# url-kaist/Quatro

Hardware: AMD Instinct MI355X
Metric: scan-pair registrations/sec (KITTI 64-ch, ~5k corr) + rot/trans err vs ref (higher is better)
Workload: dtype f32 (voxel grid, FPFH, 33-D matching: f16-split MFMA filter, exact f32 decision) / f64 (consistency graph, GNC-TLS, COTE); 1 GPU; composite: qtr_register_pair_corr per step on a synthetic KITTI-64-shaped scan pair (voxel 0.3 m), back end on 5000 planted correspondences, one pair at a time, inputs resident in HBM (--full: the detailed description)

## Files before the change

### include/quatro_hip.h

```cpp
#ifndef QUATRO_HIP_H
#define QUATRO_HIP_H

#include <stddef.h>
#include <stdint.h>

#ifdef __cplusplus
extern "C" {
#endif

#if defined(__GNUC__)
#define QTR_API __attribute__((visibility("default")))
#else
#define QTR_API
#endif

#define QTR_OK 0
#define QTR_ERR_BAD_ARG 1
#define QTR_ERR_CLIQUE_TOO_SMALL 2
#define QTR_ERR_CAPACITY 3
#define QTR_ERR_HIP 4
#define QTR_ERR_UNSUPPORTED 5
#define QTR_ERR_IO 6
#define QTR_ERR_NOT_RUN 7

// ... 286 lines not shown
QTR_API int qtr_place_index_get_info(const qtr_place_index* index, qtr_place_index_info* info);
QTR_API int qtr_place_describe(qtr_handle* h, int slot, const qtr_place_params* params, const float* xyz4, int n, float* desc,
                               int mem);
QTR_API int qtr_place_index_add(qtr_handle* h, int slot, qtr_place_index* index, const qtr_keyframe* kf, int* id_out);
QTR_API int qtr_place_index_add_desc(qtr_handle* h, int slot, qtr_place_index* index, const float* desc, int mem, int* id_out);
QTR_API long long qtr_place_index_fetch(qtr_handle* h, const qtr_place_index* index, int id, int what, void* dst, size_t bytes);
QTR_API int qtr_place_query(qtr_handle* h, int slot, const qtr_place_index* index, const qtr_keyframe* query, int id_lo,
                            int id_hi, int k, qtr_place_match* out, int* n_out);
QTR_API int qtr_place_query_desc(qtr_handle* h, int slot, const qtr_place_index* index, const float* desc, int mem, int id_lo,
                                 int id_hi, int k, qtr_place_match* out, int* n_out);

#define QTR_EVAL_MAX_PAIRS 64
typedef struct qtr_eval_params {
  double max_correspondence_distance;
  int reserved[2];
} qtr_eval_params;
typedef struct qtr_eval_result {
  int status, valid, n_source, n_corr, n_plane, reserved;
  double T[16];
  double overlap, sum_d2, inlier_rmse, plane_rmse, information[36], hessian_plane[36];
} qtr_eval_result;
typedef struct qtr_eval_kf_pair {
  const qtr_keyframe* source;
  const qtr_keyframe* target;
  double T[16];
} qtr_eval_kf_pair;
QTR_API void qtr_default_eval_params(qtr_eval_params* p);
QTR_API int qtr_evaluate(qtr_handle* h, int slot, const float* src4, int n_s, const float* tgt4, int n_t,
                         const float* tgt_normals4, const double T[16], const qtr_eval_params* prm, qtr_eval_result* res, int mem);
QTR_API int qtr_evaluate_pair(qtr_handle* h, int slot, const double T[16], const qtr_eval_params* prm, qtr_eval_result* res);
QTR_API int qtr_evaluate_keyframes(qtr_handle* h, int slot, const qtr_keyframe* source, const qtr_keyframe* target,
                                   const double T[16], const qtr_eval_params* prm, qtr_eval_result* res);
QTR_API int qtr_evaluate_keyframes_batch(qtr_handle* h, int slot, const qtr_eval_kf_pair* pairs, int B,
                                         const qtr_eval_params* prm, qtr_eval_result* results);

#define QTR_PGO_MAX_NODES 65536
#define QTR_PGO_MAX_EDGES (1 << 20)
#define QTR_PGO_MAX_ITERATIONS 65536
#define QTR_PGO_STOP_MAX_ITERATIONS 1
#define QTR_PGO_STOP_RELATIVE 2
#define QTR_PGO_STOP_STEP 3
#define QTR_PGO_STOP_LAMBDA 4
#define QTR_PGO_STOP_NOTHING 5
typedef struct qtr_pgo_params {
  int max_iterations;
  int pcg_max_iterations;
  double rel_tol;
  double step_tol;
  double tau;
  double pcg_tol;
  double line_process_weight;
  double edge_prune_threshold;
  int reserved[8];
} qtr_pgo_params;
typedef struct qtr_pgo_result {
  int status, valid, iterations, accepted, pcg_iterations_total, stop_reason, n_pruned, reserved;
  double objective_initial, objective_final, lambda_final;
} qtr_pgo_result;
QTR_API void qtr_default_pgo_params(qtr_pgo_params* p);
QTR_API int qtr_pgo_optimize(qtr_handle* h, int slot, int n_nodes, const double* poses, const unsigned char* fixed, int n_edges,
                             const int* src, const int* dst, const double* Z, const double* info,
                             const unsigned char* uncertain, const qtr_pgo_params* prm, double* poses_out, double* weight_out,
                             qtr_pgo_result* res);

#define QTR_DBG_GRAPH_BITMAP 1
#define QTR_DBG_CORE 2
#define QTR_DBG_PERM 3
#define QTR_DBG_NBR_OFFSETS 4
#define QTR_DBG_NBR_INDEX 5
#define QTR_DBG_NBR_DIST2 6
#define QTR_DBG_SPFH 7
#define QTR_DBG_NN_LARGE_OF_SMALL 8
#define QTR_DBG_NN_SMALL_OF_LARGE 9
#define QTR_DBG_VOX_SRC 10
#define QTR_DBG_VOX_TGT 11
#define QTR_DBG_CORR 12
#define QTR_DBG_MATCH_STATS 13
#define QTR_DBG_SOLVER_STATE 14
#define QTR_DBG_ICP_CORR 15
#define QTR_DBG_ICP_TRACE 16
#define QTR_DBG_ICP_TIMES 17
#define QTR_DBG_EVAL_CORR 18
#define QTR_DBG_PGO_TRACE 19
QTR_API long long qtr_debug_fetch(qtr_handle* h, int slot, int what, void* dst, size_t bytes);

QTR_API int qtr_debug_math(qtr_handle* h, int fn, const float* a, const float* b, float* out, int n);

#ifdef __cplusplus
}
#endif
#endif
```

### quatro_amd/csrc/capi.hip

```cpp
#include <dlfcn.h>

#include <algorithm>
#include <atomic>
#include <memory>
#include <mutex>
#include <new>
#include <thread>
#include <vector>

#include "common.h"
#include "frontend.h"
#include "solver.h"

struct RcclIdByValue {
  char internal[QTR_COMM_ID_BYTES];
};

struct Slot {
  hipStream_t stream = nullptr;
  hipStream_t stream2 = nullptr;
  hipEvent_t ev[8] = {};
  hipEvent_t ev_vox = nullptr;
  hipStream_t stream3 = nullptr;
  hipEvent_t ev_be0 = nullptr;
  hipEvent_t ev_end = nullptr;
  hipEvent_t ev_fork = nullptr;
  hipEvent_t ev_join = nullptr;
  void* solver_arena = nullptr;
  void* front_arena = nullptr;
  SolverBufs sb;
  FrontBufs fb;
  float4* in_src = nullptr;
  float4* in_tgt = nullptr;
  float4* m_src = nullptr;
  float4* m_tgt = nullptr;
  int* pinned_i32 = nullptr;
  qtr_result* pinned_res = nullptr;
  SegBufs seg;
  void* seg_arena = nullptr;
  ExactBufs exb;
  void* ex_arena = nullptr;
  size_t ex_bytes = 0;
  PwBufs pwb;
  void* pw_arena = nullptr;
  int* mail = nullptr;
  int seq = 0;
  unsigned long long exact_nodes = 0;
  int exact_aborted = 0;
  int times_pending = 0;
  int nn_pending = 0;
  int nn_timed_last = 0;
  long long n_matches = 0;
  float nn_dir_ms[2] = {0, 0};
  double nn_total_ms = 0;
  long long nn_total_launches = 0;
  qtr_stage_times times = {};
  int last_L = 0;
  int last_Wb = 0;
  int last_n = 0;
  int last_ns = 0, last_nt = 0;
  IcpBufs icp;
  EvalBufs eval;
  PgoBufs pgo;
  int reg_ready = 0;
  double reg_T[16] = {};
  int icp_ns = 0, icp_iters = 0;
  float icp_ms[2] = {0, 0};
  PlaceScratch place;
  KfGatherMember* merge_pin = nullptr;
  KfGatherMember* merge_dev = nullptr;
};

enum LanePhase { LANE_IDLE = 0, LANE_VOXELS, LANE_MATCH, LANE_SOLVE, LANE_REFINE_BOXES, LANE_REFINE_ITER };

struct Lane {
  int first_slot = 0, cap = 0;
  ViewStage stage;
  LanePhase phase = LANE_IDLE;
  int first_pair = 0, count = 0;
  std::vector<int> active;
  std::vector<int> ns, nt, L;
  std::vector<int> corr_only;
  std::vector<const float4*> csrc, ctgt;
  std::vector<const float4*> raw_s, raw_t;
  std::vector<int> Ps, Pt;
  bool long_lists = false;
  std::vector<IcpView> iv;
  const IcpView* ref_views = nullptr;
  int ref_it = 0, ref_nchunk = 1;
};
struct qtr_keyframe {
  qtr_handle* owner = nullptr;
  void* dev = nullptr;
  qtr_keyframe_info info = {};
};

struct qtr_place_index {
  qtr_handle* owner = nullptr;
  float* dev = nullptr;
  int stride = 0;
  qtr_place_index_info info = {};
};

struct qtr_voxel_map;

struct BatchJob {
  const qtr_pair_desc* pairs = nullptr;
  int B = 0, next = 0, done = 0;
  qtr_frontend_params fp;
  qtr_params prm;
  qtr_result* results = nullptr;
  int mem = QTR_MEM_HOST;
  bool active = false;
  std::vector<unsigned char> finished;
  bool refine = false;
  qtr_icp_params icp;
  qtr_icp_result* refined = nullptr;
  std::vector<unsigned char> ref_state;
  bool kf = false;
  std::vector<qtr_pair_desc> kf_shadow;
};

struct qtr_handle {
  int device = 0;
  qtr_limits lim;
  std::vector<Slot> slots;
  std::vector<Lane> lanes;
  BatchJob job;
  void* comm = nullptr;
  int comm_rank = 0, comm_world = 1;
  void* comm_buf = nullptr;
  size_t comm_bytes = 0;
  std::atomic<int> solves_in_flight{0};
  int spin_wait = 1;
  bool pre_on = false;
  qtr_pw_params pre_pw;
  qtr_ip_params pre_ip;
  std::atomic<bool> long_lists{false};
  struct Callers {
    std::atomic<int> live{0};
  };
  std::shared_ptr<Callers> callers = std::make_shared<Callers>();
  std::mutex share_mu;
  int share_val = 1, share_gen = 0;
  std::atomic<int> gen_inflight[4] = {};
  unsigned long long uid = 0;
  int stage_events = 1;
  int corr_overlap = 1;
  int nn_event_stride = 1;
  int icp_block = 0;
  std::mutex kf_mu;
  std::vector<qtr_keyframe*> keyframes;
  std::vector<qtr_place_index*> place_indexes;
// ... 375 lines not shown
}

int qtr_create(int device, const qtr_limits* limits, qtr_handle** out) {
  if (!out) return QTR_ERR_BAD_ARG;
  *out = nullptr;
  qtr_handle* h = new (std::nothrow) qtr_handle();
  if (!h) return QTR_ERR_CAPACITY;
  h->err[0] = 0;
  h->device = device;
  h->uid = g_handle_uid.fetch_add(1, std::memory_order_relaxed) + 1;
  {
    const char* hw = getenv("QTR_HOST_WAIT");
    h->spin_wait = (hw && strcmp(hw, "block") == 0) ? 0 : 1;
    const char* se = getenv("QTR_STAGE_EVENTS");
    h->stage_events = (se && atoi(se) == 0) ? 0 : 1;
    h->nn_event_stride = h->stage_events ? 1 : 0;
    const char* co = getenv("QTR_CORR_OVERLAP");
    h->corr_overlap = (co && atoi(co) == 0) ? 0 : 1;
    const char* ib = getenv("QTR_ICP_BLOCK");
    h->icp_block = ib ? std::max(0, atoi(ib)) : 0;
  }
  if (limits)
    h->lim = *limits;
  else
    qtr_default_limits(&h->lim);
  if (h->lim.max_points < 64 || h->lim.max_voxels < 64 || h->lim.max_corr < 64 || h->lim.n_slots < 1 ||
      h->lim.max_corr > 32768 || h->lim.max_voxels > h->lim.max_points || h->lim.max_long_neighbors < 0 ||
      h->lim.max_voxels > QTR_NN_MAX_ROWS) {
    delete h;
    return QTR_ERR_BAD_ARG;
  }
  if (h->lim.max_long_neighbors == 0)
    h->lim.max_long_neighbors = (int)std::min<long long>(128LL * h->lim.max_voxels, 1LL << 30);
  h->lim.max_long_neighbors = (h->lim.max_long_neighbors + 63) & ~63;
  h->slots.resize((size_t)h->lim.n_slots);
  const int rc = create_impl(h);
  *out = h;
  return rc;
}

static void flush_nn_totals(Slot& s) {
  if (!s.nn_pending) return;
  s.nn_pending = 0;
  float a = 0, b = 0;
  if (hipEventElapsedTime(&a, s.fb.ev_nn[0], s.fb.ev_nn[1]) == hipSuccess &&
      hipEventElapsedTime(&b, s.fb.ev_nn[2], s.fb.ev_nn[3]) == hipSuccess) {
    s.nn_total_ms += (double)a + (double)b;
    s.nn_total_launches += 2;
  }
  (void)hipGetLastError();
}

static void fill_nn_times(Slot& s) {
  float a = 0, b = 0;
  s.nn_dir_ms[0] = s.nn_dir_ms[1] = 0.f;
  if (!s.nn_timed_last) return;
  if (hipEventElapsedTime(&a, s.fb.ev_nn[0], s.fb.ev_nn[1]) == hipSuccess &&
      hipEventElapsedTime(&b, s.fb.ev_nn[2], s.fb.ev_nn[3]) == hipSuccess) {
    s.times.nn_kernel = a + b;
    s.times.nn_launches = 2;
    s.nn_dir_ms[0] = a;
    s.nn_dir_ms[1] = b;
  }
}

static bool mail_payload_ok(const Slot& s, int idx, int seq) {
  auto line_ok = [&](int base) {
    const volatile int* l = s.mail + base;
    int x = 0;
    for (int i = 0; i < 15; ++i) x ^= l[i];
    return l[15] == (seq ^ x ^ MAIL_TAG_SALT);
  };
  auto solver_ok = [&]() {
    const volatile int* m = s.mail + MAIL_SOLVER;
    int x = 0, y = 0;
    for (int i = 0; i < (int)(sizeof(qtr_result) / 4); ++i) x ^= m[i];
    for (int i = 0; i < (int)(sizeof(SolverState) / 4); ++i) y ^= m[64 + i];
    return m[63] == (seq ^ x ^ MAIL_TAG_SALT) && m[96] == (seq ^ y ^ MAIL_TAG_SALT);
  };
  switch (idx) {
    case MAIL_SEQ_VOX0: return line_ok(MAIL_VOX0);
    case MAIL_SEQ_VOX1: return line_ok(MAIL_VOX1);
    case MAIL_SEQ_MATCH: return line_ok(MAIL_MATCH) && line_ok(MAIL_CNT0) && line_ok(MAIL_CNT1);
    case MAIL_SEQ_SOLVE: return solver_ok();
    case MAIL_SEQ_ICP_BOX: return line_ok(MAIL_ICP_BOX);
    case MAIL_SEQ_ICP: return line_ok(MAIL_ICP) && line_ok(MAIL_ICP + 16) && line_ok(MAIL_ICP + 32);
    default: return true;
  }
}
static bool mail_ready(const Slot& s, int idx, int seq) {
  if (__atomic_load_n((volatile int*)(s.mail + idx), __ATOMIC_ACQUIRE) != seq) return false;
  __atomic_thread_fence(__ATOMIC_ACQUIRE);
  return mail_payload_ok(s, idx, seq);
}

static int wait_mail(qtr_handle* h, Slot& s, int idx, int seq) {
  volatile int* p = s.mail + idx;
  if (!h->spin_wait) {
    QTR_HIP_TRY(h, hipStreamSynchronize(s.stream));
  } else {
    for (unsigned long spins = 1;; ++spins) {
      if (__atomic_load_n(p, __ATOMIC_ACQUIRE) == seq) break;
      if ((spins & 0xffff) == 0) {
        const hipError_t q = hipStreamQuery(s.stream);
        if (q == hipSuccess) break;
        if (q != hipErrorNotReady) QTR_HIP_TRY(h, q);
        (void)hipGetLastError();
      }
      __builtin_ia32_pause();
    }
  }
  if (__atomic_load_n(p, __ATOMIC_ACQUIRE) != seq) {
    snprintf(h->err, sizeof(h->err), "mailbox word %d holds %d, expected %d (phase kernel did not run)", idx, (int)*p, seq);
    return QTR_ERR_HIP;
  }
  auto payload_ok = [&]() { return mail_payload_ok(s, idx, seq); };
  bool drained = false;
  for (unsigned long spins = 1;; ++spins) {
    __atomic_thread_fence(__ATOMIC_ACQUIRE);
    if (payload_ok()) return QTR_OK;
    if ((spins & 0x3fff) == 0) {
      if (drained) break;
      const hipError_t q = hipStreamSynchronize(s.stream);
      if (q != hipSuccess) QTR_HIP_TRY(h, q);
      drained = true;
    }
    __builtin_ia32_pause();
  }
  snprintf(h->err, sizeof(h->err), "mailbox payload of word %d does not match its tag (sequence %d)", idx, seq);
  return QTR_ERR_HIP;
}

static void compute_times(Slot& s) {
  if (!s.times_pending) return;
  float ms = 0;
  if (s.times_pending == 4) {
    s.times = qtr_stage_times{};
    fill_nn_times(s);
    (void)hipGetLastError();
    s.times_pending = 0;
    return;
  }
  if (s.times_pending == 3) {
    (void)hipEventSynchronize(s.ev[7]);
    s.times = qtr_stage_times{};
    if (hipEventElapsedTime(&ms, s.ev[0], s.ev[1]) == hipSuccess) s.times.voxelize = ms;
    if (hipEventElapsedTime(&ms, s.ev[1], s.ev[6]) == hipSuccess) s.times.fpfh = ms;
    if (hipEventElapsedTime(&ms, s.ev[6], s.ev[7]) == hipSuccess) s.times.match = ms;
    if (hipEventElapsedTime(&ms, s.ev[0], s.ev[7]) == hipSuccess) s.times.total = ms;
    fill_nn_times(s);
    (void)hipGetLastError();
    s.times_pending = 0;
    return;
  }
  if (s.times_pending == 6) {
    (void)hipEventSynchronize(s.ev_end);
    s.times = qtr_stage_times{};
    if (hipEventElapsedTime(&ms, s.ev[0], s.ev[1]) == hipSuccess) s.times.voxelize = ms;
    if (hipEventElapsedTime(&ms, s.ev[1], s.ev[6]) == hipSuccess) s.times.fpfh = ms;
    if (hipEventElapsedTime(&ms, s.ev[6], s.ev[7]) == hipSuccess) s.times.match = ms;
    if (hipEventElapsedTime(&ms, s.ev_be0, s.ev[2]) == hipSuccess) s.times.graph = ms;
    if (hipEventElapsedTime(&ms, s.ev[2], s.ev[3]) == hipSuccess) s.times.clique = ms;
    if (hipEventElapsedTime(&ms, s.ev[3], s.ev[4]) == hipSuccess) s.times.solve = ms;
    if (hipEventElapsedTime(&ms, s.ev[0], s.ev_end) == hipSuccess) s.times.total = ms;
    fill_nn_times(s);
    (void)hipGetLastError();
// ... 152 lines not shown
  return std::max(ncell_s, ncell_t);
}

struct ThreadCallerList {
  struct Entry {
    unsigned long long uid;
    std::shared_ptr<qtr_handle::Callers> c;
  };
  std::vector<Entry> e;
  ~ThreadCallerList() {
    for (Entry& x : e) x.c->live.fetch_sub(1, std::memory_order_acq_rel);
  }
  void enter(qtr_handle* h) {
    for (const Entry& x : e)
      if (x.uid == h->uid) return;
    if (e.size() >= 64) {
      size_t victim = 0;
      for (size_t i = 0; i < e.size(); ++i)
        if (e[i].c.use_count() == 1) {
          victim = i;
          break;
        }
      e[victim].c->live.fetch_sub(1, std::memory_order_acq_rel);
      e.erase(e.begin() + (long)victim);
    }
    h->callers->live.fetch_add(1, std::memory_order_acq_rel);
    e.push_back(Entry{h->uid, h->callers});
  }
};

struct InFlight {
  qtr_handle* h;
  int gen;
  explicit InFlight(qtr_handle* h_) : h(h_) {
    static thread_local ThreadCallerList t_callers;
    t_callers.enter(h);
    const int want = std::max(1, std::min(h->callers->live.load(std::memory_order_acquire), (int)h->slots.size()));
    bool changed = false;
    {
      std::lock_guard<std::mutex> lk(h->share_mu);
      if (want != h->share_val) {
        h->share_val = want;
        ++h->share_gen;
        changed = true;
      }
      gen = h->share_gen;
      h->gen_inflight[gen & 3].fetch_add(1, std::memory_order_acq_rel);
    }
    h->solves_in_flight.fetch_add(1, std::memory_order_acq_rel);
    if (changed)
      for (int back = 1; back <= 3; ++back)
        for (int spins = 0; h->gen_inflight[(gen - back) & 3].load(std::memory_order_acquire) > 0 && spins < 2000000; ++spins)
          std::this_thread::yield();
    solver_set_hca_share(want);
  }
  ~InFlight() {
    h->gen_inflight[gen & 3].fetch_sub(1, std::memory_order_acq_rel);
    h->solves_in_flight.fetch_sub(1, std::memory_order_acq_rel);
  }
};

static int solve_followup(qtr_handle* h, Slot& s, const float4* c_src, const float4* c_tgt, int L, const qtr_params* prm,
                          hipStream_t st, bool record_ev4) {
  if (L <= 0) return QTR_OK;
  const SolverState* ms = (const SolverState*)(s.mail + MAIL_SOLVER + 64);
  if (!ms->done) {
    s.sb.mail_seq = ++s.seq;
    QTR_HIP_TRY(h, solver_continue(s.sb, c_src, c_tgt, L, *prm, st, s.pinned_i32 + 128, ms->redo_cores));
    if (record_ev4) QTR_HIP_TRY(h, hipEventRecord(s.ev[4], st));
    QTR_TRY(wait_mail(h, s, MAIL_SEQ_SOLVE, s.seq));
  }
  if (prm->inlier_selection_mode != QTR_INLIER_PMC_EXACT) return QTR_OK;
  SolverState hs;
  memcpy(&hs, ms, sizeof(hs));
  bool improved = false;
  QTR_TRY(exact_phase(h, s, L, hs, &improved, prm->max_clique_time_limit));
  if (!improved) return QTR_OK;
  s.sb.mail_seq = ++s.seq;
  QTR_HIP_TRY(h, solver_refinalize(s.sb, c_src, c_tgt, L, *prm, st));
  if (record_ev4) QTR_HIP_TRY(h, hipEventRecord(s.ev[4], st));
  return wait_mail(h, s, MAIL_SEQ_SOLVE, s.seq);
}

static void result_from_mail(const Slot& s, qtr_result* res) {
  const int keep_ns = res->n_src, keep_nt = res->n_tgt, keep_nc = res->n_corr;
  memcpy(res, s.mail + MAIL_SOLVER, sizeof(qtr_result));
  res->n_src = keep_ns;
  res->n_tgt = keep_nt;
  res->n_corr = keep_nc;
}

static int corr_stage(qtr_handle* h, Slot& s, const float* src4, const float* tgt4, int n, int mem, hipStream_t st,
                      const float4** cs, const float4** ct) {
  *cs = (const float4*)src4;
  *ct = (const float4*)tgt4;
  if (mem != QTR_MEM_HOST) return QTR_OK;
  if (n > 0) {
    QTR_HIP_TRY(h, hipMemcpyAsync(s.m_src, src4, (size_t)n * 16, hipMemcpyHostToDevice, st));
    QTR_HIP_TRY(h, hipMemcpyAsync(s.m_tgt, tgt4, (size_t)n * 16, hipMemcpyHostToDevice, st));
  }
  *cs = s.m_src;
  *ct = s.m_tgt;
  return QTR_OK;
}

static int solve_device(qtr_handle* h, Slot& s, const float4* d_src, const float4* d_tgt, int L, const qtr_params* prm,
                        qtr_result* res, bool reset_done = false) {
  s.last_L = L;
  s.last_Wb = (((L + 63) / 64) + 3) & ~3;
  s.sb.mail_seq = ++s.seq;
  InFlight in_flight(h);
  QTR_HIP_TRY(h, solver_enqueue(s.sb, d_src, d_tgt, L, *prm, s.stream, s.pinned_i32, h->stage_events ? s.ev[2] : nullptr,
                                h->stage_events ? s.ev[3] : nullptr, reset_done));
  if (h->stage_events) QTR_HIP_TRY(h, hipEventRecord(s.ev[4], s.stream));
  QTR_TRY(wait_mail(h, s, MAIL_SEQ_SOLVE, s.seq));
  QTR_TRY(solve_followup(h, s, d_src, d_tgt, L, prm, s.stream, h->stage_events != 0));
  result_from_mail(s, res);
  return res->status;
}

static int copy_out_lists(qtr_handle* h, Slot& s, const qtr_result* res, int* clique, int* rot_inliers,
                          int* final_inliers, int cap, int mem) {
  const hipMemcpyKind kind = (mem == QTR_MEM_DEVICE) ? hipMemcpyDeviceToDevice : hipMemcpyDeviceToHost;
  if (clique && res->n_clique > 0) {
    if (res->n_clique > cap) return QTR_ERR_CAPACITY;
    QTR_HIP_TRY(h, hipMemcpyAsync(clique, s.sb.clique, sizeof(int) * (size_t)res->n_clique, kind, s.stream));
  }
  if (rot_inliers && res->n_rot_inliers > 0) {
    if (res->n_rot_inliers > cap) return QTR_ERR_CAPACITY;
    QTR_HIP_TRY(h, hipMemcpyAsync(rot_inliers, s.sb.rot_inl, sizeof(int) * (size_t)res->n_rot_inliers, kind, s.stream));
  }
  if (final_inliers && res->n_final > 0) {
    if (res->n_final > cap) return QTR_ERR_CAPACITY;
    QTR_HIP_TRY(h, hipMemcpyAsync(final_inliers, s.sb.final_inl, sizeof(int) * (size_t)res->n_final, kind, s.stream));
  }
  QTR_HIP_TRY(h, hipStreamSynchronize(s.stream));
  return QTR_OK;
}

int qtr_solve(qtr_handle* h, int slot, const float* src4, const float* tgt4, int L, const qtr_params* prm,
              qtr_result* res, int* clique, int* rot_inliers, int* final_inliers, int cap, int mem) {
  Slot* sp = get_slot(h, slot);
  if (!sp || !res) return QTR_ERR_BAD_ARG;
  Slot& s = *sp;
  memset(res, 0, sizeof(*res));
  int rc = check_params(h, prm);
  if (rc != QTR_OK) return res->status = rc;
  if (L < 0 || (L > 0 && (!src4 || !tgt4))) {
    snprintf(h->err, sizeof(h->err), "bad input clouds");
    return res->status = QTR_ERR_BAD_ARG;
  }
  if ((rc = check_max_corr(h, L)) != QTR_OK) return res->status = rc;
  QTR_HIP_TRY(h, hipSetDevice(h->device));
  const float4 *d_src = nullptr, *d_tgt = nullptr;
  const bool ev_on = h->stage_events != 0;
  if (ev_on) QTR_HIP_TRY(h, hipEventRecord(s.ev[0], s.stream));
  QTR_TRY(corr_stage(h, s, src4, tgt4, L, mem, s.stream, &d_src, &d_tgt));
  if (ev_on) QTR_HIP_TRY(h, hipEventRecord(s.ev[1], s.stream));
  res->n_corr = L;
  rc = solve_device(h, s, d_src, d_tgt, L, prm, res);
  if (rc != QTR_OK && rc != QTR_ERR_CLIQUE_TOO_SMALL) return rc;
  s.times_pending = ev_on ? 1 : 4;
  const int rc2 = copy_out_lists(h, s, res, clique, rot_inliers, final_inliers, cap, mem);
  if (rc2 != QTR_OK) return res->status = rc2;
  return rc;
}

int qtr_max_clique(qtr_handle* h, int slot, const unsigned long long* adj, int L, int mode, double kcore_thr,
                   double time_limit, int* clique, int cap, int* n_out, int* max_core_out, int mem) {
  Slot* sp = get_slot(h, slot);
  if (!sp || !n_out || L < 0 || (L > 0 && (!adj || !clique))) return QTR_ERR_BAD_ARG;
  Slot& s = *sp;
  *n_out = 0;
  if (max_core_out) *max_core_out = 0;
  if (mode != QTR_INLIER_PMC_HEU && mode != QTR_INLIER_KCORE_HEU && mode != QTR_INLIER_PMC_EXACT) {
    snprintf(h->err, sizeof(h->err), "clique solver mode %d not supported", mode);
    return QTR_ERR_UNSUPPORTED;
  }
  QTR_TRY(check_max_corr(h, L));
  if (L == 0) return QTR_OK;
  QTR_HIP_TRY(h, hipSetDevice(h->device));
  const int W = (L + 63) / 64;
  const u64* d_adj = (const u64*)adj;
  if (mem == QTR_MEM_HOST) {
    QTR_HIP_TRY(h, hipMemcpyAsync(s.sb.bm, adj, (size_t)L * W * 8, hipMemcpyHostToDevice, s.stream));
    d_adj = s.sb.bm;
  }
  s.last_L = L;
  s.last_Wb = (L + 63) / 64;
  InFlight in_flight(h);
  QTR_HIP_TRY(h, clique_only_enqueue(s.sb, d_adj, L, mode, kcore_thr, s.stream));
  QTR_HIP_TRY(h, hipMemcpyAsync(s.pinned_i32 + 128, s.sb.st, sizeof(SolverState), hipMemcpyDeviceToHost, s.stream));
  QTR_HIP_TRY(h, hipStreamSynchronize(s.stream));
  if (!((const SolverState*)(s.pinned_i32 + 128))->done) {
    qtr_params dummy;
    qtr_default_params(&dummy);
    QTR_HIP_TRY(h, solver_continue(s.sb, nullptr, nullptr, L, dummy, s.stream, s.pinned_i32 + 128,
                                   ((const SolverState*)(s.pinned_i32 + 128))->redo_cores));
  }
  if (mode == QTR_INLIER_PMC_EXACT) {
    SolverState hs;
    memcpy(&hs, s.pinned_i32 + 128, sizeof(hs));
    bool improved = false;
    QTR_TRY(exact_phase(h, s, L, hs, &improved, time_limit));
  }
  s.sb.mail_seq = ++s.seq;
  QTR_HIP_TRY(h, clique_only_finish(s.sb, L, s.stream));
  QTR_TRY(wait_mail(h, s, MAIL_SEQ_SOLVE, s.seq));
  memcpy(s.pinned_res, s.mail + MAIL_SOLVER, sizeof(qtr_result));
  const int M = s.pinned_res->n_clique;
  if (max_core_out) *max_core_out = s.pinned_res->max_core;
  *n_out = M;
  if (M > cap) return QTR_ERR_CAPACITY;
  if (M > 0) {
    const hipMemcpyKind kind = (mem == QTR_MEM_DEVICE) ? hipMemcpyDeviceToDevice : hipMemcpyDeviceToHost;
    QTR_HIP_TRY(h, hipMemcpyAsync(clique, s.sb.clique, sizeof(int) * (size_t)M, kind, s.stream));
    QTR_HIP_TRY(h, hipStreamSynchronize(s.stream));
  }
  return QTR_OK;
}

static bool stage_fits(qtr_handle* h, Slot& s, size_t doubles, size_t ints) {
  if (doubles <= (size_t)72 * s.sb.Lcap && ints <= (size_t)24 * s.sb.Lcap) return true;
  snprintf(h->err, sizeof(h->err), "stage call needs %zu doubles / %zu ints of scratch; raise max_corr (now %d)",
           doubles, ints, s.sb.Lcap);
  return false;
}

int qtr_compute_tims(qtr_handle* h, int slot, const double* v3n, int N, double* tims3k, int* map2k) {
  Slot* sp = get_slot(h, slot);
  if (!sp || N < 0 || (N > 1 && (!v3n || !tims3k || !map2k))) return QTR_ERR_BAD_ARG;
  Slot& s = *sp;
  const long long K = (long long)N * (N - 1) / 2;
  if (K <= 0) return QTR_OK;
  if (!stage_fits(h, s, (size_t)3 * N + (size_t)3 * K, (size_t)2 * K)) return QTR_ERR_CAPACITY;
  QTR_HIP_TRY(h, hipSetDevice(h->device));
  double* d_v = s.sb.f64;
  double* d_t = d_v + (size_t)3 * N;
  QTR_HIP_TRY(h, hipMemcpyAsync(d_v, v3n, sizeof(double) * 3 * (size_t)N, hipMemcpyHostToDevice, s.stream));
  hipLaunchKernelGGL(k_compute_tims, dim3((unsigned)((K + 255) / 256)), dim3(256), 0, s.stream, d_v, N, K, d_t, s.sb.i32);
  QTR_HIP_TRY(h, hipGetLastError());
  QTR_HIP_TRY(h, hipMemcpyAsync(tims3k, d_t, sizeof(double) * 3 * (size_t)K, hipMemcpyDeviceToHost, s.stream));
  QTR_HIP_TRY(h, hipMemcpyAsync(map2k, s.sb.i32, sizeof(int) * 2 * (size_t)K, hipMemcpyDeviceToHost, s.stream));
  QTR_HIP_TRY(h, hipStreamSynchronize(s.stream));
  return QTR_OK;
}
// ... 418 lines not shown
  const float4* d_in = (const float4*)xyz4;
  if (mem == QTR_MEM_HOST) {
    QTR_HIP_TRY(h, hipMemcpyAsync(s.in_src, xyz4, (size_t)P * 16, hipMemcpyHostToDevice, s.stream));
    d_in = s.in_src;
  }
  QTR_HIP_TRY(h, hipEventRecord(s.ev[0], s.stream));
  CloudBufs& cb = s.fb.cloud[0];
  {
    const float4* raws[1] = {d_in};
    const int Ps[1] = {P};
    QTR_HIP_TRY(h, voxelize_enqueue(s.fb, 1, raws, Ps, leaf, s.stream));
  }
  QTR_HIP_TRY(h, hipEventRecord(s.ev[1], s.stream));
  QTR_HIP_TRY(h, hipMemcpyAsync(s.pinned_i32, cb.counts, 16 * sizeof(int), hipMemcpyDeviceToHost, s.stream));
  QTR_HIP_TRY(h, hipStreamSynchronize(s.stream));
  const VoxVerdict v = vox_verdict(s.pinned_i32, P, h->lim.max_voxels);
  if (v.reason == VOX_TIMEOUT || s.pinned_i32[CNT_VOX_TAILERR]) {
    snprintf(h->err, sizeof(h->err), "voxel grid: look-back timed out");
    return QTR_ERR_HIP;
  }
  const int n = v.n;
  const float4* d_out = v.passed ? d_in : cb.vox;
  if (v.reason == VOX_TOO_MANY) {
    snprintf(h->err, sizeof(h->err), "voxel count %d exceeds max_voxels=%d", n, h->lim.max_voxels);
    return QTR_ERR_CAPACITY;
  }
  if (n > cap) {
    snprintf(h->err, sizeof(h->err), "voxel count %d exceeds output capacity %d", n, cap);
    *n_out = n;
    return QTR_ERR_CAPACITY;
  }
  QTR_HIP_TRY(h, hipMemcpyAsync(out_xyz4, d_out, (size_t)n * 16,
                                mem == QTR_MEM_HOST ? hipMemcpyDeviceToHost : hipMemcpyDeviceToDevice, s.stream));
  QTR_HIP_TRY(h, hipStreamSynchronize(s.stream));
  *n_out = n;
  times_one_stage(s, &qtr_stage_times::voxelize);
  return QTR_OK;
}

int qtr_fpfh(qtr_handle* h, int slot, const float* xyz4, int n, float r_normal, float r_fpfh, float* normals4,
             float* desc33, int mem) {
  Slot* sp = get_slot(h, slot);
  if (!sp || n < 0 || (n > 0 && (!xyz4 || !desc33))) return QTR_ERR_BAD_ARG;
  if (r_normal > r_fpfh || !(r_normal > 0)) {
    snprintf(h->err, sizeof(h->err), "[FPFHManager]: Normal should be lower than fpfh_radius!!!!");
    return QTR_ERR_BAD_ARG;
  }
  Slot& s = *sp;
  s.last_n = n;
  if (n == 0) return QTR_OK;
  if (n > h->lim.max_voxels) {
    snprintf(h->err, sizeof(h->err), "n=%d exceeds max_voxels=%d", n, h->lim.max_voxels);
    return QTR_ERR_CAPACITY;
  }
  QTR_HIP_TRY(h, hipSetDevice(h->device));
  CloudBufs& cb = s.fb.cloud[0];
  const hipMemcpyKind kin = mem == QTR_MEM_HOST ? hipMemcpyHostToDevice : hipMemcpyDeviceToDevice;
  const hipMemcpyKind kout = mem == QTR_MEM_HOST ? hipMemcpyDeviceToHost : hipMemcpyDeviceToDevice;
  QTR_HIP_TRY(h, hipMemcpyAsync(cb.vox, xyz4, (size_t)n * 16, kin, s.stream));
  QTR_HIP_TRY(h, hipMemsetAsync(cb.counts, 0, 16 * sizeof(int), s.stream));
  QTR_HIP_TRY(h, set_count_enqueue(cb, CNT_NVOX, n, s.stream));
  QTR_HIP_TRY(h, hipEventRecord(s.ev[0], s.stream));
  {
    const int ns1[1] = {n};
    QTR_TRY(ensure_long_arenas(h, s));
    QTR_HIP_TRY(h, fpfh_enqueue(s.fb, 0, 1, ns1, r_normal, r_fpfh, s.stream, true, false, true));
  }
  QTR_HIP_TRY(h, hipEventRecord(s.ev[1], s.stream));
  QTR_HIP_TRY(h, hipMemcpyAsync(s.pinned_i32, cb.counts, 16 * sizeof(int), hipMemcpyDeviceToHost, s.stream));
  QTR_HIP_TRY(h, hipStreamSynchronize(s.stream));
  if (s.pinned_i32[CNT_NBR_CAPACITY]) {
    snprintf(h->err, sizeof(h->err), "radius-neighbour lists longer than %d entries need %d entries of the long-list arena "
             "(longest list %d); qtr_limits.max_long_neighbors is %d", QTR_KMAX, s.pinned_i32[CNT_NBR_ARENA],
             s.pinned_i32[CNT_KMAX], h->lim.max_long_neighbors);
    return QTR_ERR_CAPACITY;
  }
  if (normals4) QTR_HIP_TRY(h, hipMemcpyAsync(normals4, cb.normals, (size_t)n * 16, kout, s.stream));
  QTR_HIP_TRY(h, hipMemcpyAsync(desc33, cb.fpfh, (size_t)n * 33 * 4, kout, s.stream));
  QTR_HIP_TRY(h, hipStreamSynchronize(s.stream));
  times_one_stage(s, &qtr_stage_times::fpfh);
  return QTR_OK;
}

static int match_device(qtr_handle* h, Slot& s, int ns, int nt, const qtr_frontend_params* fp, int* L_out,
                        bool init_done = false, bool prep_done = false, bool tolerate_tail = false, bool gather = true) {
  flush_nn_totals(s);
  const int stride = h->nn_event_stride;
  s.fb.nn_events = (stride > 0 && (s.n_matches++ % stride) == 0) ? 1 : 0;
  s.nn_timed_last = (s.fb.nn_events && s.fb.nn_engine != 0) ? 1 : 0;
  s.nn_pending = s.nn_timed_last;
  s.fb.mail_seq = ++s.seq;
  QTR_HIP_TRY(h, match_enqueue(s.fb, ns, nt, *fp, s.stream, init_done, prep_done, gather));
  QTR_TRY(wait_mail(h, s, MAIL_SEQ_MATCH, s.seq));
  *L_out = s.mail[MAIL_MATCH + MC_NCORR];
  if (*L_out < 0) {
    if (tolerate_tail) return QTR_OK;
    *L_out = 0;
    (void)hipStreamSynchronize(s.stream);
    snprintf(h->err, sizeof(h->err), "matcher tail: look-back timed out (no correspondences were written)");
    return QTR_ERR_HIP;
  }
  return QTR_OK;
}

int qtr_match(qtr_handle* h, int slot, const float* xyz4_s, int n_s, const float* desc33_s, const float* xyz4_t,
              int n_t, const float* desc33_t, const qtr_frontend_params* fp, int* corr2, int cap, int* L_out, int mem) {
  Slot* sp = get_slot(h, slot);
  if (!sp || !fp || !L_out || n_s < 0 || n_t < 0) return QTR_ERR_BAD_ARG;
  Slot& s = *sp;
  *L_out = 0;
  s.last_ns = n_s;
  s.last_nt = n_t;
  if (n_s == 0 || n_t == 0) return QTR_OK;
  if (!xyz4_s || !xyz4_t || !desc33_s || !desc33_t || !corr2) return QTR_ERR_BAD_ARG;
  if (n_s > h->lim.max_voxels || n_t > h->lim.max_voxels) {
    snprintf(h->err, sizeof(h->err), "cloud size exceeds max_voxels=%d", h->lim.max_voxels);
    return QTR_ERR_CAPACITY;
  }
  QTR_HIP_TRY(h, hipSetDevice(h->device));
  const hipMemcpyKind kin = mem == QTR_MEM_HOST ? hipMemcpyHostToDevice : hipMemcpyDeviceToDevice;
  const hipMemcpyKind kout = mem == QTR_MEM_HOST ? hipMemcpyDeviceToHost : hipMemcpyDeviceToDevice;
  QTR_HIP_TRY(h, hipMemcpyAsync(s.fb.cloud[0].vox, xyz4_s, (size_t)n_s * 16, kin, s.stream));
  QTR_HIP_TRY(h, hipMemcpyAsync(s.fb.cloud[1].vox, xyz4_t, (size_t)n_t * 16, kin, s.stream));
  QTR_HIP_TRY(h, hipMemcpyAsync(s.fb.cloud[0].fpfh, desc33_s, (size_t)n_s * 132, kin, s.stream));
  QTR_HIP_TRY(h, hipMemcpyAsync(s.fb.cloud[1].fpfh, desc33_t, (size_t)n_t * 132, kin, s.stream));
  QTR_HIP_TRY(h, hipEventRecord(s.ev[0], s.stream));
  {
    const int n2[2] = {n_s, n_t};
    QTR_HIP_TRY(h, mean_enqueue(s.fb, 0, 2, n2, s.stream));
  }
  int L = 0;
  int rc = match_device(h, s, n_s, n_t, fp, &L);
  if (rc != QTR_OK) return rc;
  QTR_HIP_TRY(h, hipEventRecord(s.ev[1], s.stream));
  *L_out = L;
  if (L > cap) {
    snprintf(h->err, sizeof(h->err), "L=%d exceeds output capacity %d", L, cap);
    return QTR_ERR_CAPACITY;
  }
  if (L > 0) QTR_HIP_TRY(h, hipMemcpyAsync(corr2, s.fb.corr, (size_t)L * 8, kout, s.stream));
  QTR_HIP_TRY(h, hipStreamSynchronize(s.stream));
  times_one_stage(s, &qtr_stage_times::match);
  fill_nn_times(s);
  return QTR_OK;
}

static int ensure_stream3(qtr_handle* h, Slot& s) {
  if (s.stream3) return QTR_OK;
  int prio_least = 0, prio_greatest = 0;
  QTR_HIP_TRY(h, hipDeviceGetStreamPriorityRange(&prio_least, &prio_greatest));
  if (!s.ev_be0) QTR_HIP_TRY(h, hipEventCreate(&s.ev_be0));
  if (!s.ev_end) QTR_HIP_TRY(h, hipEventCreate(&s.ev_end));
  if (!s.ev_fork) QTR_HIP_TRY(h, hipEventCreateWithFlags(&s.ev_fork, hipEventDisableTiming));
  if (!s.ev_join) QTR_HIP_TRY(h, hipEventCreateWithFlags(&s.ev_join, hipEventDisableTiming));
  if (prio_greatest != prio_least) QTR_HIP_TRY(h, hipStreamCreateWithPriority(&s.stream3, hipStreamNonBlocking, prio_least));
  else QTR_HIP_TRY(h, hipStreamCreateWithFlags(&s.stream3, hipStreamNonBlocking));
  return QTR_OK;
}

struct CorrEarly {
  const float* src = nullptr;
  const float* tgt = nullptr;
  int n = 0, mem = QTR_MEM_HOST;
  const qtr_params* prm = nullptr;
  bool enqueued = false;
  int seq = 0;
  const float4 *cs = nullptr, *ct = nullptr;
  std::unique_ptr<InFlight> in_flight;
};
static int corr_early_enqueue(qtr_handle* h, Slot& s, CorrEarly& ce) {
  ce.enqueued = true;
  const bool ev_on = h->stage_events != 0;
  QTR_HIP_TRY(h, hipStreamWaitEvent(s.stream3, s.ev_fork, 0));
  if (ev_on) QTR_HIP_TRY(h, hipEventRecord(s.ev_be0, s.stream3));
  QTR_TRY(corr_stage(h, s, ce.src, ce.tgt, ce.n, ce.mem, s.stream3, &ce.cs, &ce.ct));
  s.last_L = ce.n;
  s.last_Wb = (((ce.n + 63) / 64) + 3) & ~3;
  s.sb.mail_seq = ce.seq = ++s.seq;
  ce.in_flight.reset(new InFlight(h));
  QTR_HIP_TRY(h, solver_enqueue(s.sb, ce.cs, ce.ct, ce.n, *ce.prm, s.stream3, s.pinned_i32, ev_on ? s.ev[2] : nullptr,
                                ev_on ? s.ev[3] : nullptr, false, true));
  if (ev_on) QTR_HIP_TRY(h, hipEventRecord(s.ev[4], s.stream3));
  return QTR_OK;
}

static int front_device(qtr_handle* h, Slot& s, const float* src_raw4, int Ps, const float* tgt_raw4, int Pt,
                        const qtr_frontend_params* fp, int mem, bool for_solver, int* ns_out, int* nt_out, int* L_out,
                        bool corr_given = false, CorrEarly* early = nullptr) {
  int rc = QTR_OK;
  if (fp->normal_radius > fp->fpfh_radius) {
    snprintf(h->err, sizeof(h->err), "[FPFHManager]: Normal should be lower than fpfh_radius!!!!");
    return QTR_ERR_BAD_ARG;
  }
  if (Ps <= 0 || Pt <= 0 || !src_raw4 || !tgt_raw4) {
    snprintf(h->err, sizeof(h->err), "Invalid or empty point cloud dataset given!");
    return QTR_ERR_BAD_ARG;
  }
  if (Ps > h->lim.max_points || Pt > h->lim.max_points) {
    snprintf(h->err, sizeof(h->err), "cloud exceeds max_points=%d", h->lim.max_points);
    return QTR_ERR_CAPACITY;
  }
  QTR_HIP_TRY(h, hipSetDevice(h->device));
  if (early && !early->enqueued) {
    QTR_TRY(ensure_stream3(h, s));
    QTR_HIP_TRY(h, hipEventRecord(s.ev_fork, s.stream));
  }
  const float4 *d_s = (const float4*)src_raw4, *d_t = (const float4*)tgt_raw4;
  if (mem == QTR_MEM_HOST) {
    QTR_HIP_TRY(h, hipMemcpyAsync(s.in_src, src_raw4, (size_t)Ps * 16, hipMemcpyHostToDevice, s.stream));
    QTR_HIP_TRY(h, hipMemcpyAsync(s.in_tgt, tgt_raw4, (size_t)Pt * 16, hipMemcpyHostToDevice, s.stream));
    d_s = s.in_src;
    d_t = s.in_tgt;
  }
  if (h->stage_events) QTR_HIP_TRY(h, hipEventRecord(s.ev[0], s.stream));
  auto fail_drained = [&](int code) {
    (void)hipStreamSynchronize(s.stream);
    return code;
  };
  {
    const float4* raws[2] = {d_s, d_t};
    const int Ps2[2] = {Ps, Pt};
    for (int attempt = 0;; ++attempt) {
      const int launched = s.fb.vox_passes;
      const int vox_seq = s.fb.mail_seq = ++s.seq;
      QTR_HIP_TRY(h, voxelize_enqueue(s.fb, 2, raws, Ps2, fp->voxel_size, s.stream, launched, fp->fpfh_radius * 1.001f));
      QTR_HIP_TRY(h, hipEventRecord(s.ev_vox, s.stream));
      {
        const int on_device[2] = {-1, -1};
        QTR_HIP_TRY(h, hipStreamWaitEvent(s.stream2, s.ev_vox, 0));
        QTR_HIP_TRY(h, mean_enqueue(s.fb, 0, 2, on_device, s.stream2, h->lim.max_voxels));
      }
      if (early && !early->enqueued) QTR_TRY(corr_early_enqueue(h, s, *early));
      if ((rc = wait_mail(h, s, MAIL_SEQ_VOX0, vox_seq)) != QTR_OK || (rc = wait_mail(h, s, MAIL_SEQ_VOX1, vox_seq)) != QTR_OK)
        return fail_drained(rc);
      const int bits = std::max(s.mail[MAIL_VOX0 + CNT_SORT_BITS], s.mail[MAIL_VOX1 + CNT_SORT_BITS]);
      if (!vox_passes_next(s.fb.vox_passes, s.fb.vox_fewer, bits, launched, attempt)) break;
    }
  }
  const VoxVerdict vs = vox_verdict(s.mail + MAIL_VOX0, Ps, h->lim.max_voxels),
                   vt = vox_verdict(s.mail + MAIL_VOX1, Pt, h->lim.max_voxels);
  const int ns = vs.n, nt = vt.n;
  const bool passed_through = vs.passed || vt.passed;
  if (vs.reason == VOX_TIMEOUT || vt.reason == VOX_TIMEOUT) {
    snprintf(h->err, sizeof(h->err), "voxel grid: look-back timed out");
    return fail_drained(QTR_ERR_HIP);
  }
  if (vs.reason == VOX_PASS_TOO_LARGE || vt.reason == VOX_PASS_TOO_LARGE) {
    snprintf(h->err, sizeof(h->err), "voxel grid would overflow int32 (leaf too small): the cloud passes through as it "
             "is (pcl::VoxelGrid), and its %d / %d points exceed max_voxels=%d", Ps, Pt, h->lim.max_voxels);
    return fail_drained(QTR_ERR_CAPACITY);
  }
  if (vs.passed) QTR_HIP_TRY(h, hipMemcpyAsync(s.fb.cloud[0].vox, d_s, (size_t)Ps * 16, hipMemcpyDeviceToDevice, s.stream));
  if (vt.passed) QTR_HIP_TRY(h, hipMemcpyAsync(s.fb.cloud[1].vox, d_t, (size_t)Pt * 16, hipMemcpyDeviceToDevice, s.stream));
  if (passed_through) QTR_HIP_TRY(h, hipEventRecord(s.ev_vox, s.stream));
  if (vs.reason == VOX_TOO_MANY || vt.reason == VOX_TOO_MANY) {
    snprintf(h->err, sizeof(h->err), "voxel count (%d,%d) exceeds max_voxels=%d", ns, nt, h->lim.max_voxels);
    return fail_drained(QTR_ERR_CAPACITY);
  }
  *ns_out = ns;
  *nt_out = nt;
  s.last_ns = ns;
  s.last_nt = nt;
  if (h->stage_events) QTR_HIP_TRY(h, hipEventRecord(s.ev[1], s.stream));
  {
    const int n2[2] = {ns, nt};
    if (passed_through) {
      QTR_HIP_TRY(h, hipStreamWaitEvent(s.stream2, s.ev_vox, 0));
      QTR_HIP_TRY(h, mean_enqueue(s.fb, 0, 2, n2, s.stream2));
    }
    if (h->long_lists) QTR_TRY(ensure_long_arenas(h, s));
    QTR_HIP_TRY(h, fpfh_enqueue(s.fb, 0, 2, n2, fp->normal_radius, fp->fpfh_radius, s.stream, false, true, h->long_lists, true,
                                cell_table_cells(s.mail[MAIL_VOX0 + CNT_NCELL], s.mail[MAIL_VOX1 + CNT_NCELL])));
    QTR_HIP_TRY(h, match_init_enqueue(s.fb, ns, nt, *fp, s.stream2, false, for_solver ? (int*)s.sb.st : nullptr,
                                      (int)(sizeof(SolverState) / 4)));
    QTR_HIP_TRY(h, hipEventRecord(s.ev[5], s.stream2));
    QTR_HIP_TRY(h, hipStreamWaitEvent(s.stream, s.ev[5], 0));
  }
  if (h->stage_events) QTR_HIP_TRY(h, hipEventRecord(s.ev[6], s.stream));
  int L = 0;
  rc = match_device(h, s, ns, nt, fp, &L, true, true, corr_given, early == nullptr);
  if (rc != QTR_OK) return rc;
  switch (lists_verdict(s.mail + MAIL_CNT0, s.mail + MAIL_CNT1, h->long_lists)) {
    case LISTS_TILE_ERROR:
      snprintf(h->err, sizeof(h->err), "voxel grid: look-back timed out in a tile (centroids incomplete)");
      return QTR_ERR_HIP;
    case LISTS_CAPACITY:
      snprintf(h->err, sizeof(h->err), "radius-neighbour lists longer than %d entries (longest %d / %d) exceed the long-list "
               "arena: qtr_limits.max_long_neighbors is %d", QTR_KMAX, s.mail[MAIL_CNT0 + CNT_KMAX],
               s.mail[MAIL_CNT1 + CNT_KMAX], h->lim.max_long_neighbors);
      return QTR_ERR_CAPACITY;
    case LISTS_NEED_LONG:
      h->long_lists = true;
      return front_device(h, s, src_raw4, Ps, tgt_raw4, Pt, fp, mem, for_solver, ns_out, nt_out, L_out, corr_given, early);
    case LISTS_OK: break;
  }
  *L_out = L;
  if (corr_given) {
    if (h->stage_events) QTR_HIP_TRY(h, hipEventRecord(s.ev[7], s.stream));
    return QTR_OK;
  }
  s.last_L = L;
  QTR_TRY(check_max_corr(h, L));
  QTR_HIP_TRY(h, gather_matched_enqueue(s.fb, L, s.m_src, s.m_tgt, s.stream));
  if (h->stage_events) QTR_HIP_TRY(h, hipEventRecord(s.ev[7], s.stream));
  return QTR_OK;
}

static void mark_registration(Slot& s, int rc, const qtr_result* res) {
  if (rc != QTR_OK && rc != QTR_ERR_CLIQUE_TOO_SMALL) return;
  s.reg_ready = 1;
  for (int k = 0; k < 16; ++k) s.reg_T[k] = res->T[k];
}

static int register_pair_impl(qtr_handle* h, Slot& s, const float* src_raw4, int Ps, const float* tgt_raw4, int Pt,
                              const qtr_frontend_params* fp, const qtr_params* prm, qtr_result* res, int* clique,
                              int* final_inliers, int cap, int mem_in, int mem_out, const float* corr_src,
                              const float* corr_tgt, int n_corr, int* n_matched = nullptr) {
  const bool given = n_corr >= 0;
  int L = 0;
  if (given && h->corr_overlap) {
    CorrEarly ce;
    ce.src = corr_src;
    ce.tgt = corr_tgt;
    ce.n = n_corr;
    ce.mem = mem_out;
    ce.prm = prm;
    int rc = front_device(h, s, src_raw4, Ps, tgt_raw4, Pt, fp, mem_in, false, &res->n_src, &res->n_tgt, &L, true, &ce);
    if (n_matched) *n_matched = L;
    res->n_corr = n_corr;
    if (!ce.enqueued) return res->status = rc;
    struct DrainOnReturn {
      hipStream_t st;
      bool armed = true;
      ~DrainOnReturn() {
        if (armed) (void)hipStreamSynchronize(st);
      }
    } drain{s.stream3};
    struct StreamSwap {
      Slot& s;
      hipStream_t keep;
      StreamSwap(Slot& s_, hipStream_t st) : s(s_), keep(s_.stream) { s.stream = st; }
      ~StreamSwap() { s.stream = keep; }
    };
    if (rc == QTR_OK) {
      StreamSwap on_stream3(s, s.stream3);
      rc = wait_mail(h, s, MAIL_SEQ_SOLVE, ce.seq);
      if (rc == QTR_OK) rc = solve_followup(h, s, ce.cs, ce.ct, n_corr, prm, s.stream3, h->stage_events != 0);
    }
    if (rc != QTR_OK) {
      return res->status = rc;
    }
    ce.in_flight.reset();
    result_from_mail(s, res);
    rc = res->status;
    QTR_HIP_TRY(h, hipEventRecord(s.ev_join, s.stream3));
    QTR_HIP_TRY(h, hipStreamWaitEvent(s.stream, s.ev_join, 0));
    if (h->stage_events) QTR_HIP_TRY(h, hipEventRecord(s.ev_end, s.stream));
    if (rc != QTR_OK && rc != QTR_ERR_CLIQUE_TOO_SMALL) return rc;
    s.times_pending = h->stage_events ? 6 : 4;
    const int rc2 = copy_out_lists(h, s, res, clique, nullptr, final_inliers, cap, mem_out);
    if (rc2 != QTR_OK) return res->status = rc2;
    drain.armed = false;
    return rc;
  }
  int rc = front_device(h, s, src_raw4, Ps, tgt_raw4, Pt, fp, mem_in, true, &res->n_src, &res->n_tgt, &L, given);
  if (n_matched) *n_matched = L;
  res->n_corr = given ? n_corr : L;
  if (rc != QTR_OK) return res->status = rc;
  const float4 *cs = s.m_src, *ct = s.m_tgt;
  if (given) QTR_TRY(corr_stage(h, s, corr_src, corr_tgt, n_corr, mem_out, s.stream, &cs, &ct));
  rc = solve_device(h, s, cs, ct, res->n_corr, prm, res, true);
  if (rc != QTR_OK && rc != QTR_ERR_CLIQUE_TOO_SMALL) return rc;
  s.times_pending = h->stage_events ? 2 : 4;
  const int rc2 = copy_out_lists(h, s, res, clique, nullptr, final_inliers, cap, mem_out);
  if (rc2 != QTR_OK) return res->status = rc2;
  return rc;
}

int qtr_register_pair(qtr_handle* h, int slot, const float* src_raw4, int Ps, const float* tgt_raw4, int Pt,
                      const qtr_frontend_params* fp, const qtr_params* prm, qtr_result* res, int* clique,
                      int* final_inliers, int cap, int mem) {
  Slot* sp = get_slot(h, slot);
  if (!sp || !res || !fp) return QTR_ERR_BAD_ARG;
  memset(res, 0, sizeof(*res));
  const int rc = check_params(h, prm);
  if (rc != QTR_OK) return res->status = rc;
  const int rc2 = register_pair_impl(h, *sp, src_raw4, Ps, tgt_raw4, Pt, fp, prm, res, clique, final_inliers, cap, mem, mem,
                                     nullptr, nullptr, -1);
  mark_registration(*sp, rc2, res);
  return rc2;
}

int qtr_register_pair_corr(qtr_handle* h, int slot, const float* src_raw4, int Ps, const float* tgt_raw4, int Pt,
                           const qtr_frontend_params* fp, const float* corr_src4, const float* corr_tgt4, int n_corr,
                           const qtr_params* prm, qtr_result* res, int* n_matched, int* clique, int* final_inliers, int cap,
                           int mem) {
  Slot* sp = get_slot(h, slot);
  if (!sp || !res || !fp) return QTR_ERR_BAD_ARG;
  Slot& s = *sp;
  memset(res, 0, sizeof(*res));
  if (n_matched) *n_matched = 0;
  int rc = check_params(h, prm);
  if (rc != QTR_OK) return res->status = rc;
  if (n_corr < 0 || (n_corr > 0 && (!corr_src4 || !corr_tgt4))) {
    snprintf(h->err, sizeof(h->err), "bad correspondence clouds");
    return res->status = QTR_ERR_BAD_ARG;
  }
  if (n_corr > h->lim.max_corr) {
    snprintf(h->err, sizeof(h->err), "n_corr=%d exceeds max_corr=%d", n_corr, h->lim.max_corr);
    return res->status = QTR_ERR_CAPACITY;
  }
  rc = register_pair_impl(h, s, src_raw4, Ps, tgt_raw4, Pt, fp, prm, res, clique, final_inliers, cap, mem, mem, corr_src4,
                          corr_tgt4, n_corr, n_matched);
  mark_registration(s, rc, res);
  return rc;
}

int qtr_feature_pair(qtr_handle* h, int slot, const float* src_raw4, int Ps, const float* tgt_raw4, int Pt,
                     const qtr_frontend_params* fp, int* n_src, int* n_tgt, int* L_out, float* src_kps4, float* tgt_kps4,
                     int* corr2, int cap, int mem) {
  Slot* sp = get_slot(h, slot);
  if (!sp || !fp || !L_out) return QTR_ERR_BAD_ARG;
  Slot& s = *sp;
  int ns = 0, nt = 0, L = 0;
  *L_out = 0;
  const int rc = front_device(h, s, src_raw4, Ps, tgt_raw4, Pt, fp, mem, false, &ns, &nt, &L);
  if (n_src) *n_src = ns;
  if (n_tgt) *n_tgt = nt;
  *L_out = L;
  if (rc != QTR_OK) return rc;
  s.times_pending = h->stage_events ? 3 : 4;
  if ((src_kps4 || tgt_kps4 || corr2) && L > cap) {
    snprintf(h->err, sizeof(h->err), "L=%d exceeds output capacity %d", L, cap);
    return QTR_ERR_CAPACITY;
  }
  const hipMemcpyKind kout = mem == QTR_MEM_HOST ? hipMemcpyDeviceToHost : hipMemcpyDeviceToDevice;
  if (L > 0) {
    if (src_kps4) QTR_HIP_TRY(h, hipMemcpyAsync(src_kps4, s.m_src, (size_t)L * 16, kout, s.stream));
    if (tgt_kps4) QTR_HIP_TRY(h, hipMemcpyAsync(tgt_kps4, s.m_tgt, (size_t)L * 16, kout, s.stream));
    if (corr2) QTR_HIP_TRY(h, hipMemcpyAsync(corr2, s.fb.corr, (size_t)L * 8, kout, s.stream));
  }
  if (mem == QTR_MEM_HOST) QTR_HIP_TRY(h, hipStreamSynchronize(s.stream));
  return QTR_OK;
}

static int front_one_check(qtr_handle* h, bool have_cloud, int P, const qtr_frontend_params* fp) {
  if (fp->normal_radius > fp->fpfh_radius) {
    snprintf(h->err, sizeof(h->err), "[FPFHManager]: Normal should be lower than fpfh_radius!!!!");
    return QTR_ERR_BAD_ARG;
  }
  if (P <= 0 || !have_cloud) {
    snprintf(h->err, sizeof(h->err), "Invalid or empty point cloud dataset given!");
    return QTR_ERR_BAD_ARG;
  }
  if (P > h->lim.max_points) {
    snprintf(h->err, sizeof(h->err), "cloud exceeds max_points=%d", h->lim.max_points);
    return QTR_ERR_CAPACITY;
// ... 440 lines not shown
  if (n_out) *n_out = 0;
  Slot* sp = peek_slot(h, slot);
  if (!sp || !ix || !query || !out || !n_out) return QTR_ERR_BAD_ARG;
  if (query->owner != h) {
    snprintf(h->err, sizeof(h->err), "keyframe belongs to another handle");
    return QTR_ERR_BAD_ARG;
  }
  int lo = 0, n = 0;
  QTR_TRY(place_query_begin(h, ix, id_lo, id_hi, k, &lo, &n));
  if (n == 0) return QTR_OK;
  QTR_HIP_TRY(h, hipSetDevice(h->device));
  QTR_TRY(place_scratch_ensure(h, *sp, ix->stride, ix->info.capacity));
  QTR_HIP_TRY(h, place_describe_enqueue((const float4*)((const char*)query->dev + KF_HDR_BYTES), query->info.n_voxels,
                                        ix->info.params, sp->place.q, sp->stream));
  return place_query_finish(h, *sp, ix, lo, n, k, out, n_out);
}

int qtr_place_query_desc(qtr_handle* h, int slot, const qtr_place_index* ix, const float* desc, int mem, int id_lo, int id_hi,
                         int k, qtr_place_match* out, int* n_out) {
  if (n_out) *n_out = 0;
  Slot* sp = peek_slot(h, slot);
  if (!sp || !ix || !desc || !out || !n_out || (mem != QTR_MEM_HOST && mem != QTR_MEM_DEVICE)) return QTR_ERR_BAD_ARG;
  int lo = 0, n = 0;
  QTR_TRY(place_query_begin(h, ix, id_lo, id_hi, k, &lo, &n));
  if (n == 0) return QTR_OK;
  QTR_HIP_TRY(h, hipSetDevice(h->device));
  QTR_TRY(place_scratch_ensure(h, *sp, ix->stride, ix->info.capacity));
  const qtr_place_params& p = ix->info.params;
  QTR_HIP_TRY(h, hipMemcpyAsync(sp->place.q, desc, (size_t)p.num_rings * p.num_sectors * 4,
                                mem == QTR_MEM_HOST ? hipMemcpyHostToDevice : hipMemcpyDeviceToDevice, sp->stream));
  QTR_HIP_TRY(h, place_colnorm_enqueue(sp->place.q, p, sp->stream));
  return place_query_finish(h, *sp, ix, lo, n, k, out, n_out);
}

static int check_keyframes(qtr_handle* h, const qtr_keyframe* a, const qtr_keyframe* b, const qtr_frontend_params* fp) {
  if (!a || !b) {
    snprintf(h->err, sizeof(h->err), "keyframe is NULL");
    return QTR_ERR_BAD_ARG;
  }
  if (a->owner != h || b->owner != h) {
    snprintf(h->err, sizeof(h->err), "keyframe belongs to another handle");
    return QTR_ERR_BAD_ARG;
  }
  auto same = [](float x, float y) { return memcmp(&x, &y, 4) == 0; };
  for (const qtr_keyframe* k : {a, b})
    if (!same(k->info.voxel_size, fp->voxel_size) || !same(k->info.normal_radius, fp->normal_radius) ||
        !same(k->info.fpfh_radius, fp->fpfh_radius)) {
      snprintf(h->err, sizeof(h->err), "keyframe was made with voxel_size %g, normal_radius %g, fpfh_radius %g; the call asks "
               "for %g, %g, %g", k->info.voxel_size, k->info.normal_radius, k->info.fpfh_radius, fp->voxel_size,
               fp->normal_radius, fp->fpfh_radius);
      return QTR_ERR_BAD_ARG;
    }
  return QTR_OK;
}

int qtr_register_keyframes(qtr_handle* h, int slot, const qtr_keyframe* kf_src, const qtr_keyframe* kf_tgt,
                           const qtr_frontend_params* fp, const qtr_params* prm, qtr_result* res, int* clique,
                           int* final_inliers, int cap) {
  Slot* sp = get_slot(h, slot);
  if (!sp || !res || !fp) return QTR_ERR_BAD_ARG;
  Slot& s = *sp;
  memset(res, 0, sizeof(*res));
  int rc = check_params(h, prm);
  if (rc != QTR_OK) return res->status = rc;
  if ((rc = check_keyframes(h, kf_src, kf_tgt, fp)) != QTR_OK) return res->status = rc;
  QTR_HIP_TRY(h, hipSetDevice(h->device));
  const int ns = kf_src->info.n_voxels, nt = kf_tgt->info.n_voxels;
  res->n_src = s.last_ns = ns;
  res->n_tgt = s.last_nt = nt;
  if (h->stage_events) QTR_HIP_TRY(h, hipEventRecord(s.ev[0], s.stream));
  QTR_HIP_TRY(h, match_init_enqueue(s.fb, ns, nt, *fp, s.stream, true, (int*)s.sb.st, (int)(sizeof(SolverState) / 4)));
  QTR_HIP_TRY(h, kf_load_enqueue(s.fb, kf_src->dev, ns, kf_tgt->dev, nt, s.stream));
  int L = 0;
  rc = match_device(h, s, ns, nt, fp, &L, true, true);
  res->n_corr = L;
  if (rc != QTR_OK) return res->status = rc;
  s.last_L = L;
  if ((rc = check_max_corr(h, L)) != QTR_OK) return res->status = rc;
  QTR_HIP_TRY(h, gather_matched_enqueue(s.fb, L, s.m_src, s.m_tgt, s.stream));
  if (h->stage_events) QTR_HIP_TRY(h, hipEventRecord(s.ev[7], s.stream));
  rc = solve_device(h, s, s.m_src, s.m_tgt, L, prm, res, true);
  if (rc != QTR_OK && rc != QTR_ERR_CLIQUE_TOO_SMALL) return rc;
  s.times_pending = h->stage_events ? 5 : 4;
  const int rc2 = copy_out_lists(h, s, res, clique, nullptr, final_inliers, cap, QTR_MEM_HOST);
  if (rc2 != QTR_OK) return res->status = rc2;
  mark_registration(s, rc, res);
  return rc;
}

static void batch_fail_pair(qtr_handle* h, int pair, int status) {
  qtr_result& r = h->job.results[pair];
  r.status = status;
  r.valid = 0;
  h->job.finished[pair] = 1;
  ++h->job.done;
}

static int check_icp_params(qtr_handle* h, const qtr_icp_params* p);
static int icp_device(qtr_handle* h, Slot& s, const float4* d_src, int ns, const float4* d_tgt, int nt, const float4* d_nrm,
                      const float4* d_src_nrm, const double* guess, const qtr_icp_params* prm, qtr_icp_result* res);

static void refine_fill_rest(qtr_handle* h, bool failed) {
  BatchJob& J = h->job;
  if (!J.refine) return;
  for (int i = 0; i < J.B; ++i) {
    if (J.ref_state[i] == 2) continue;
    qtr_icp_result& q = J.refined[i];
    memset(&q, 0, sizeof(q));
    q.status = QTR_ERR_NOT_RUN;
    if (failed && !J.finished[i]) q.status = J.results[i].status;
    else if (failed && J.ref_state[i] == 1) q.status = QTR_ERR_HIP;
    for (int k = 0; k < 16; ++k) q.T[k] = J.results[i].T[k];
    J.ref_state[i] = 2;
  }
}

static void batch_abort(qtr_handle* h) {
  BatchJob& J = h->job;
  for (auto& ln : h->lanes) {
    Slot& lead = h->slots[ln.first_slot];
    (void)hipStreamSynchronize(lead.stream);
    (void)hipStreamSynchronize(lead.stream2);
    ln.phase = LANE_IDLE;
  }
  (void)hipGetLastError();
  for (int i = 0; i < J.B; ++i) {
    if (J.finished[i]) continue;
    memset(&J.results[i], 0, sizeof(qtr_result));
    J.results[i].status = i < J.next ? QTR_ERR_HIP : QTR_ERR_NOT_RUN;
  }
  refine_fill_rest(h, true);
  J.active = false;
}

static inline bool pair_has_scans(const qtr_pair_desc& pd) { return pd.src_raw4 != nullptr || pd.tgt_raw4 != nullptr; }
static inline bool pair_has_corr(const qtr_pair_desc& pd) {
  return pd.src_corr4 != nullptr || pd.tgt_corr4 != nullptr || pd.n_corr != 0;
}

static int lane_start_chunk(qtr_handle* h, Lane& ln);
static int lane_enqueue_refine(qtr_handle* h, Lane& ln);

static int lane_enqueue_solver(qtr_handle* h, Lane& ln, const std::vector<int>& from_match) {
  BatchJob& J = h->job;
  Slot& lead = h->slots[ln.first_slot];
  std::vector<int> all(from_match);
  all.insert(all.end(), ln.corr_only.begin(), ln.corr_only.end());
  ln.corr_only.clear();
  ln.active.swap(all);
  if (ln.active.empty()) return lane_start_chunk(h, ln);
  std::vector<int> Ls;
  std::vector<SolverBufs*> SB;
  std::vector<const float4*> srcs, tgts;
  for (int g : ln.active) {
    Slot& s = h->slots[ln.first_slot + g];
    s.last_L = ln.L[g];
    s.last_Wb = (((ln.L[g] + 63) / 64) + 3) & ~3;
    s.sb.mail_seq = ++s.seq;
    SB.push_back(&s.sb);
    srcs.push_back(ln.csrc[g]);
    tgts.push_back(ln.ctgt[g]);
    Ls.push_back(ln.L[g]);
  }
  solver_set_hca_share((int)h->lanes.size());
  QTR_HIP_TRY(h, solver_enqueue_group(SB.data(), (int)SB.size(), srcs.data(), tgts.data(), Ls.data(), J.prm, &ln.stage,
                                      lead.stream));
  ln.phase = LANE_SOLVE;
// ... 1303 lines not shown
    QTR_HIP_TRY(h, hipMemcpyAsync((void*)v.off, off.data(), (n + 1) * 4, hipMemcpyHostToDevice, st));
    QTR_HIP_TRY(h, hipMemcpyAsync((void*)v.inc, inc.data(), 2 * e * 4, hipMemcpyHostToDevice, st));
    QTR_HIP_TRY(h, hipMemcpyAsync((void*)v.Z, Z, e * 128, hipMemcpyHostToDevice, st));
    QTR_HIP_TRY(h, hipMemcpyAsync((void*)v.info, info, e * 288, hipMemcpyHostToDevice, st));
    for (int k = 0; k < 2; ++k) QTR_HIP_TRY(h, hipMemcpyAsync(v.X[k], poses, n * 128, hipMemcpyHostToDevice, st));
    QTR_HIP_TRY(h, hipMemcpyAsync(v.st, &P.pin[0], sizeof(QtrPgoState), hipMemcpyHostToDevice, st));
    QTR_HIP_TRY(h, hipMemsetAsync(v.ticket, 0, 64, st));
    const QtrPgoState& now = P.pin[1];
    for (int it = 0; it <= cfg.max_iterations; ++it) {
      hipLaunchKernelGGL(k_pgo_linearize, dim3(qtr_div_up(E, 256)), dim3(256), 0, st, v);
      hipLaunchKernelGGL(k_pgo_step, dim3(1), dim3(QTR_PGO_THREADS), 0, st, v);
      QTR_HIP_TRY(h, hipGetLastError());
      QTR_HIP_TRY(h, hipMemcpyAsync(&P.pin[1], v.st, sizeof(QtrPgoState), hipMemcpyDeviceToHost, st));
      QTR_HIP_TRY(h, hipStreamSynchronize(st));
      if (now.stop) break;
    }
    if (!now.stop) {
      snprintf(h->err, sizeof(h->err), "qtr_pgo_optimize: the device did not stop after %d iterations", cfg.max_iterations);
      return QTR_ERR_HIP;
    }
    QTR_HIP_TRY(h, hipMemcpyAsync(poses_out, v.X[now.cur], n * 128, hipMemcpyDeviceToHost, st));
    std::vector<double> w(e);
    QTR_HIP_TRY(h, hipMemcpyAsync(w.data(), v.Ew[now.cur], e * 8, hipMemcpyDeviceToHost, st));
    QTR_HIP_TRY(h, hipStreamSynchronize(st));
    P.last_rows = 1 + now.trials;
    res->iterations = now.trials;
    res->accepted = now.accepted;
    res->pcg_iterations_total = now.pcg_total;
    res->stop_reason = now.reason;
    res->objective_initial = now.F0;
    res->objective_final = now.F;
    res->lambda_final = now.lambda;
    res->valid = pgo_finite(now.F) ? 1 : 0;
    for (int k = 0; k < E; ++k) {
      if (un[k] && w[k] < prm->edge_prune_threshold) res->n_pruned += 1;
      if (weight_out) weight_out[k] = w[k];
    }
    return QTR_OK;
  }();
  return res->status = rc;
}

long long qtr_debug_fetch(qtr_handle* h, int slot, int what, void* dst, size_t bytes) {
  Slot* sp = peek_slot(h, slot);
  if (!sp) return -1;
  Slot& s = *sp;
  if (hipSetDevice(h->device) != hipSuccess) return -1;
  const void* src = nullptr;
  size_t have = 0;
  const int L = s.last_L, W = (L + 63) / 64;
  CloudBufs& c0 = s.fb.cloud[0];
  switch (what) {
    case QTR_DBG_GRAPH_BITMAP: src = s.sb.bm; have = (size_t)L * W * 8; break;
    case QTR_DBG_CORE: src = s.sb.core; have = (size_t)L * 4; break;
    case QTR_DBG_PERM: src = s.sb.perm; have = (size_t)L * 4; break;
    case QTR_DBG_NBR_OFFSETS:
      if (exclusive_scan_i32(c0.nbr_cnt, c0.nbr_off, s.last_n, s.stream) != hipSuccess) return -1;
      src = c0.nbr_off;
      have = (size_t)(s.last_n + 1) * 4;
      break;
    case QTR_DBG_NBR_INDEX:
    case QTR_DBG_NBR_DIST2: {
      int tot = 0;
      if (exclusive_scan_i32(c0.nbr_cnt, c0.nbr_off, s.last_n, s.stream) != hipSuccess) return -1;
      if (hipStreamSynchronize(s.stream) != hipSuccess) return -1;
      if (hipMemcpy(&tot, c0.nbr_off + s.last_n, 4, hipMemcpyDeviceToHost) != hipSuccess) return -1;
      src = (what == QTR_DBG_NBR_INDEX) ? (const void*)c0.nbr_idx : (const void*)c0.nbr_d2;
      have = (size_t)tot * 4;
      break;
    }
    case QTR_DBG_SPFH: src = c0.spfh; have = (size_t)s.last_n * 132; break;
    case QTR_DBG_NN_LARGE_OF_SMALL: src = s.fb.nn_of_small; have = (size_t)(s.last_ns < s.last_nt ? s.last_ns : s.last_nt) * 4; break;
    case QTR_DBG_NN_SMALL_OF_LARGE: src = s.fb.nn_of_large; have = (size_t)(s.last_ns < s.last_nt ? s.last_nt : s.last_ns) * 4; break;
    case QTR_DBG_VOX_SRC: src = s.fb.cloud[0].vox; have = (size_t)s.last_ns * 16; break;
    case QTR_DBG_VOX_TGT: src = s.fb.cloud[1].vox; have = (size_t)s.last_nt * 16; break;
    case QTR_DBG_CORR: src = s.fb.corr; have = (size_t)s.last_L * 8; break;
    case QTR_DBG_MATCH_STATS: src = s.fb.mcounts; have = 16 * 4; break;
    case QTR_DBG_SOLVER_STATE: src = s.sb.st; have = sizeof(SolverState); break;
    case QTR_DBG_ICP_CORR: src = s.icp.v.corr; have = s.icp.v.corr ? (size_t)s.icp_ns * 4 : 0; break;
    case QTR_DBG_ICP_TRACE: src = s.icp.v.trace; have = s.icp.v.trace ? (size_t)s.icp_iters * 18 * 8 : 0; break;
    case QTR_DBG_ICP_TIMES: src = s.icp_ms; have = sizeof(s.icp_ms); break;
    case QTR_DBG_EVAL_CORR: src = s.eval.last_corr; have = s.eval.last_corr ? (size_t)s.eval.last_ns * 4 : 0; break;
    case QTR_DBG_PGO_TRACE: src = s.pgo.last_trace; have = s.pgo.last_trace ? (size_t)s.pgo.last_rows * QTR_PGO_TRACE * 8 : 0; break;
    default: return -1;
  }
  const size_t n = have < bytes ? have : bytes;
  if (dst && n > 0) {
    if (hipStreamSynchronize(s.stream) != hipSuccess) return -1;
    if (what == QTR_DBG_GRAPH_BITMAP && s.last_Wb > W) {
      const size_t rows = n / ((size_t)W * 8);
      if (rows > 0 && hipMemcpy2D(dst, (size_t)W * 8, src, (size_t)s.last_Wb * 8, (size_t)W * 8, rows, hipMemcpyDeviceToHost) !=
                          hipSuccess)
        return -1;
    } else if (what == QTR_DBG_ICP_TIMES) {
      memcpy(dst, src, n);
    } else if (hipMemcpy(dst, src, n, hipMemcpyDeviceToHost) != hipSuccess) {
      return -1;
    }
  }
  return (long long)have;
}

__global__ void k_debug_math(int fn, const float* a, const float* b, float* out, int n) {
  const int i = blockIdx.x * blockDim.x + threadIdx.x;
  if (i >= n) return;
  float r = 0.f, s, c;
  switch (fn) {
    case 0: r = qm_atan2f(a[i], b[i]); break;
    case 1: r = qm_acosf(a[i]); break;
    case 2: qm_sincosf(a[i], &s, &c); r = s; break;
    case 3: qm_sincosf(a[i], &s, &c); r = c; break;
    case 5: r = spfh_swap_roles(a[i], b[i]) ? 1.f : 0.f; break;
    default: break;
  }
  out[i] = r;
}

int qtr_debug_math(qtr_handle* h, int fn, const float* a, const float* b, float* out, int n) {
  if (!h || !a || !out || n <= 0) return QTR_ERR_BAD_ARG;
  QTR_HIP_TRY(h, hipSetDevice(h->device));
  float *da = nullptr, *db = nullptr, *dout = nullptr;
  QTR_HIP_TRY(h, hipMalloc((void**)&da, (size_t)n * 4));
  QTR_HIP_TRY(h, hipMalloc((void**)&db, (size_t)n * 4));
  QTR_HIP_TRY(h, hipMalloc((void**)&dout, (size_t)n * 4));
  QTR_HIP_TRY(h, hipMemcpy(da, a, (size_t)n * 4, hipMemcpyHostToDevice));
  QTR_HIP_TRY(h, hipMemcpy(db, b ? b : a, (size_t)n * 4, hipMemcpyHostToDevice));
  hipLaunchKernelGGL(k_debug_math, dim3((n + 255) / 256), dim3(256), 0, 0, fn, da, db, dout, n);
  QTR_HIP_TRY(h, hipGetLastError());
  QTR_HIP_TRY(h, hipMemcpy(out, dout, (size_t)n * 4, hipMemcpyDeviceToHost));
  (void)hipFree(da);
  (void)hipFree(db);
  (void)hipFree(dout);
  return QTR_OK;
}

}
```

### quatro_amd/csrc/frontend.h

```cpp
#pragma once
#include "common.h"
#include "front_verdict.h"

#define QTR_KMAX 256
#define NBIG_LDS_KEYS 8192
#define RADIX_TILE 1024
#define NORM_BINS 192

#define QTR_NN_MAX_ROWS ((1 << 20) - 32)
#define QTR_CELL_CAP (1 << 21)
enum { MC_NCORR = 0, MC_HIDDEN_I = 1, MC_HIDDEN_J = 2, MC_NCROSS = 3, MC_NTUPLE = 4, MC_SWAPPED = 5, MC_NQ0 = 6, MC_NHIT = 7,
       MC_RECHECK0 = 8, MC_RECHECK1 = 9, MC_NSPLIT0 = 10, MC_NSPLIT1 = 11 ,
       MC_UNSAFE = 12,
       MC_TAILERR = 13  };

enum { MAIL_VOX0 = 0, MAIL_VOX1 = 16, MAIL_MATCH = 32, MAIL_CNT0 = 48, MAIL_CNT1 = 64, MAIL_SEQ_VOX0 = 96, MAIL_SEQ_VOX1 = 97,
       MAIL_SEQ_MATCH = 98, MAIL_SEQ_SOLVE = 99, MAIL_SEQ_ICP_BOX = 100, MAIL_SEQ_ICP = 101, MAIL_SOLVER = 128,
       MAIL_ICP_BOX = 256, MAIL_ICP = 272, MAIL_INTS = 512 };

struct CloudBufs {
  int* counts = nullptr;
  u32* mm = nullptr;
  u32* mm_part = nullptr;
  float4* vox = nullptr;
  float4* normals = nullptr;
  float* spfh = nullptr;
  float* fpfh = nullptr;
  u64* keys_a = nullptr;
  u64* keys_b = nullptr;
  u32* hist = nullptr;
  int* vox_look = nullptr;
  int* nbr_cnt = nullptr;
  int* nbr_off = nullptr;
  int* nbr_idx = nullptr;
  float* nbr_d2 = nullptr;
  int* nbr_big_idx = nullptr;
  float* nbr_big_d2 = nullptr;
  int nbr_big_cap = 0;
  float4* spts = nullptr;
  float4* raw_sorted = nullptr;
  int* ranges = nullptr;
  int* cell_cnt = nullptr;
  int* cell_start = nullptr;
  float* mean = nullptr;
  float* baseT = nullptr;
  float* queryT = nullptr;
  float* norms = nullptr;
  u32* max_norm = nullptr;
  float* baseTb = nullptr;
  int* nb_row = nullptr;
  int* nb_start = nullptr;
  uint4* baseH = nullptr;
  uint4* queryH = nullptr;
  u64* dd_hash = nullptr;
  u64* dd_table = nullptr;
};

struct CloudView {
  const float4* raw;
  int P;
  int n;
  int* counts;
  u32* mm;
  u32* mm_part;
  float4* vox;
  float4* normals;
  float* spfh;
  float* fpfh;
  u64* keys_a;
  u64* keys_b;
  u32* hist;
  int* mail;
  int* mail_seq_slot;
  int seq;
  int* blkcnt;
  int* blkoff;
  int* vox_look;
  int* nbr_cnt;
  int* nbr_off;
  int* nbr_idx;
  float* nbr_d2;
  int* nbr_big_idx;
  float* nbr_big_d2;
  int nbr_big_cap;
  float4* spts;
  int* ranges;
  int* cell_cnt;
  int* cell_start;
  float* mean;
  float* norms;
  u64* dd_hash;
  u64* dd_table;
  int dd_mask;
};
struct Clouds2 {
  CloudView c[2];
  const CloudView* ext;
};

struct NnDir {
// ... 14 lines not shown
  const int* bstart;
  const int* qorder;
  u64* best;
  int nq_slot, rc_slot;
};
struct NnPartial {
  float b1, b2;
  int i1;
  int pad;
};
#define TAIL_MAXWG 256
struct MatchView {
  NnDir d[2];
  const float4 *vox_i, *vox_j;
  const float *mean_i, *mean_j;
  const float *fpfh_i, *fpfh_j;
  float *baseT_i, *queryT_i, *norms_i, *baseT_j, *queryT_j, *norms_j;
  float *baseTb_i, *baseTb_j;
  uint4 *baseH_i, *baseH_j, *queryH_i, *queryH_j, *queryH_c;
  int *nb_row_i, *nb_row_j, *nb_start_i, *nb_start_j;
  u64 *hash_i, *hash_j, *table_i, *table_j;
  int dd_mask;
  int n_large, n_small, pad_large, pad_small, swapped, ns, nt;
  u64 *best_small, *best_large;
  int *nn_of_small, *nn_of_large, *cross_i, *cross_j, *flags, *scan, *passed, *tgt_of_src, *corr, *mcounts;
  NnPartial* partial;
  int* recheck_rows;
  float* recheck_thr;
  int2* recheck_span;
  int* recheck_q;
  int* hit_rows;
  float* queryT_c;
  float* norms_c;
  const float4 *vox_s, *vox_t;
  float4 *m_src, *m_tgt;
  int m_cap;
  int* mail;
  const int *counts0, *counts1;
  int seq;
  int *nc_cnt, *nc_fill, *nc_off, *nc_list;
  int crosscheck;
  int tuple;
  float tuple_scale;
  u64 seed;
};
struct MatchArgs {
  MatchView one;
  const MatchView* ext;
};

struct FrontBufs {
  int max_points = 0, max_voxels = 0;
  CloudBufs cloud[2];
  u64* best_small = nullptr;
  u64* best_large = nullptr;
  int* nn_of_small = nullptr;
  int* nn_of_large = nullptr;
  int* cross_i = nullptr;
  int* cross_j = nullptr;
  int* flags = nullptr;
  int* scan = nullptr;
  int* passed = nullptr;
  int* tgt_of_src = nullptr;
  int* corr = nullptr;
  int* mcounts = nullptr;
  void* nn_partial = nullptr;
  int* recheck_rows = nullptr;
  float* recheck_thr = nullptr;
  int2* recheck_span = nullptr;
  int* recheck_q = nullptr;
  int* hit_rows = nullptr;
  float* queryT_c = nullptr;
  float* norms_c = nullptr;
  uint4* queryH_c = nullptr;
  int dd_slots = 0;
  int *nc_cnt = nullptr, *nc_fill = nullptr, *nc_off = nullptr, *nc_list = nullptr;
  int* mail = nullptr;
  float4* m_src = nullptr;
  float4* m_tgt = nullptr;
  int m_cap = 0;
  int vox_passes = 4;
  int vox_fewer = 0;
  bool gathered = false;
  int mail_seq = 0;
  int nn_engine = 2;
  int n_cu = 256;
  int nn_events = 1;
  hipEvent_t ev_nn[4] = {};
};

size_t frontend_scratch_bytes(int max_points, int max_voxels);
void frontend_carve(FrontBufs& F, void* base, int max_points, int max_voxels);
hipError_t frontend_init_attributes();

hipError_t voxelize_enqueue(FrontBufs& F, int nc, const float4* const* raw, const int* P, float leaf, hipStream_t st,
                            int passes = 4, float cell_side = 0.f);
hipError_t set_count_enqueue(CloudBufs& C, int which, int value, hipStream_t st);
hipError_t fpfh_enqueue(FrontBufs& F, int first, int nc, const int* n, float r_normal, float r_fpfh, hipStream_t st,
                        bool with_mean, bool origin_known, bool long_lists, bool desc_prep = false,
                        int max_ncell = 0 );
hipError_t mean_enqueue(FrontBufs& F, int first, int nc, const int* n, hipStream_t st, int cap = 0);
hipError_t match_enqueue(FrontBufs& F, int ns, int nt, const qtr_frontend_params& fp, hipStream_t st, bool init_done = false,
                         bool prep_done = false, bool gather = true);
hipError_t match_init_enqueue(FrontBufs& F, int ns, int nt, const qtr_frontend_params& fp, hipStream_t st,
                              bool clear_tables, int* zero_words = nullptr, int n_zero = 0);
hipError_t gather_matched_enqueue(FrontBufs& F, int L, float4* m_src, float4* m_tgt, hipStream_t st);

hipError_t voxelize_enqueue_group(FrontBufs* const* F, int G, const float4* const* raw, const int* P, float leaf,
                                  ViewStage* stage, hipStream_t st, float cell_side = 0.f);
hipError_t mean_enqueue_group(FrontBufs* const* F, int G, const int* n, ViewStage* stage, hipStream_t st);
hipError_t fpfh_enqueue_group(FrontBufs* const* F, int G, const int* n, float r_normal, float r_fpfh, ViewStage* stage,
                              hipStream_t st, bool long_lists, bool desc_prep = false, int max_ncell = 0);
hipError_t match_enqueue_group(FrontBufs* const* F, int G, const int* n, const qtr_frontend_params* fp,
                               const unsigned long long* seeds, ViewStage* stage, hipStream_t st, bool prep_done = false);

hipError_t exclusive_scan_i32(const int* in, int* out, int n, hipStream_t st);
```

### quatro_amd/csrc/frontend.hip

```cpp
#include <stdlib.h>

#include <type_traits>
#include <vector>

#include "common.h"
#include "frontend.h"

__device__ __forceinline__ u32 enc_f32(float f) {
  const u32 b = __float_as_uint(f);
  return (b & 0x80000000u) ? ~b : (b | 0x80000000u);
}
__device__ __forceinline__ float dec_f32(u32 e) {
  const u32 b = (e & 0x80000000u) ? (e & 0x7fffffffu) : ~e;
  return __uint_as_float(b);
}


__global__ void k_set_count(int* counts, int which, int value) {
  if (threadIdx.x == 0 && blockIdx.x == 0) counts[which] = value;
}

__device__ __forceinline__ void d_minmax(const float4* __restrict__ pts, int n, u32* __restrict__ part) {
  float mn[3] = {INFINITY, INFINITY, INFINITY}, mx[3] = {-INFINITY, -INFINITY, -INFINITY};
  for (int i = blockIdx.x * blockDim.x + threadIdx.x; i < n; i += gridDim.x * blockDim.x) {
// ... 1708 lines not shown
  per_cloud += 4096 + MM_MAX_PARTS * 32 + 256;
  per_cloud += (size_t)max_voxels * (16 + 16 + 132 + 132);
  per_cloud += 2 * (size_t)max_points * 8;
  per_cloud += (size_t)(4096 * ((max_points + RADIX_TILE - 1) / RADIX_TILE) + 8192) * 4 + 65536;
  per_cloud += (size_t)((max_points + RADIX_TILE - 1) / RADIX_TILE + 64) * 4 * (RADIX_TILE / VOX_TILE_SINGLE) + 256;
  per_cloud += (size_t)max_voxels * 4 * 2 + 64;
  per_cloud += (size_t)max_voxels * QTR_KMAX * 8;
  per_cloud += (size_t)max_voxels * (16 + 72) + 512;
  per_cloud += 2 * (size_t)(QTR_CELL_CAP + 4096) * 4 + 512;
  per_cloud += (size_t)max_points * 16 + 256;
  size_t shared = (size_t)max_voxels * 64 + 16384 + 2 * TAIL_MAXWG * 4;
  shared += (size_t)max_voxels * (4 + 4 + 4 + 8) + (size_t)max_voxels * 4 * 6 + 4096;
  const size_t vpad = ((size_t)max_voxels + 511) / 512 * 512;
  per_cloud += 3 * 34 * vpad * 4 + (size_t)max_voxels * 8 + 4096;
  per_cloud += 2 * (vpad * 224 + 2 * 7168) + 512;
  per_cloud += (size_t)max_voxels * 8 + (size_t)dedup_slots(max_voxels) * 8 + 512;
  shared += vpad * 32 * 16 + 4 * ((size_t)max_voxels * 4 + 1024);
  shared += (size_t)max_voxels * 4 + 34 * vpad * 4 + vpad * 4 + 1024;
  shared += vpad * 224 + 2 * 7168 + 256 + (size_t)max_voxels * 4 + 1024;
  return 2 * per_cloud + shared + 64 * 256;
}

void frontend_carve(FrontBufs& F, void* base, int max_points, int max_voxels) {
  char* p = (char*)base;
  auto take = [&](size_t bytes) {
    char* r = p;
    p += (bytes + 255) & ~(size_t)255;
    return (void*)r;
  };
  F.max_points = max_points;
  F.max_voxels = max_voxels;
  for (int c = 0; c < 2; ++c) {
    CloudBufs& C = F.cloud[c];
    C.counts = (int*)take(16 * 4);
    C.mm = (u32*)take(8 * 4);
    C.mm_part = (u32*)take(MM_MAX_PARTS * 8 * 4);
    C.mean = (float*)take(4 * 4);
    C.vox = (float4*)take((size_t)max_voxels * 16);
    C.normals = (float4*)take((size_t)max_voxels * 16);
    C.spfh = (float*)take((size_t)max_voxels * 132);
    C.fpfh = (float*)take((size_t)max_voxels * 132);
    C.keys_a = (u64*)take((size_t)max_points * 8);
    C.keys_b = (u64*)take((size_t)max_points * 8);
    C.hist = (u32*)take((size_t)(4096 * ((max_points + RADIX_TILE - 1) / RADIX_TILE) + 8192) * 4);
    C.vox_look = (int*)take((size_t)((max_points + RADIX_TILE - 1) / RADIX_TILE + 64) * 4 * (RADIX_TILE / VOX_TILE_SINGLE));
    C.nbr_cnt = (int*)take((size_t)max_voxels * 4);
    C.nbr_off = (int*)take((size_t)(max_voxels + 1) * 4);
    C.nbr_idx = (int*)take((size_t)max_voxels * QTR_KMAX * 4);
    C.nbr_d2 = (float*)take((size_t)max_voxels * QTR_KMAX * 4);
    C.spts = (float4*)take((size_t)max_voxels * 16);
    C.raw_sorted = (float4*)take((size_t)max_points * 16);
    C.ranges = (int*)take((size_t)max_voxels * 18 * 4);
    C.cell_cnt = (int*)take((size_t)(QTR_CELL_CAP + 4096) * 4);
    C.cell_start = (int*)take((size_t)(QTR_CELL_CAP + 4096) * 4);
    const size_t vpad = ((size_t)max_voxels + 511) / 512 * 512;
    C.baseT = (float*)take(34 * vpad * 4);
    C.queryT = (float*)take(34 * vpad * 4);
    C.baseTb = (float*)take(34 * vpad * 4);
    C.baseH = (uint4*)take(vpad * 224 + 2 * 7168);
    C.queryH = (uint4*)take(vpad * 224 + 2 * 7168);
    C.nb_row = (int*)take((size_t)max_voxels * 4);
    C.nb_start = (int*)take((NORM_BINS + 2) * 4);
    C.norms = (float*)take((size_t)max_voxels * 4);
    C.max_norm = (u32*)take(64);
    C.dd_hash = (u64*)take((size_t)max_voxels * 8);
    C.dd_table = (u64*)take((size_t)dedup_slots(max_voxels) * 8);
  }
  F.dd_slots = dedup_slots(max_voxels);
  F.best_small = (u64*)take((size_t)max_voxels * 8);
  F.best_large = (u64*)take((size_t)max_voxels * 8);
  F.nn_of_small = (int*)take((size_t)max_voxels * 4);
  F.nn_of_large = (int*)take((size_t)max_voxels * 4);
  F.cross_i = (int*)take((size_t)max_voxels * 8);
  F.cross_j = (int*)take((size_t)max_voxels * 8);
  F.flags = (int*)take((size_t)max_voxels * 4);
  F.scan = (int*)take((size_t)max(max_voxels + 1, 2 * TAIL_MAXWG) * 4);
  F.passed = (int*)take((size_t)max_voxels * 8);
  F.tgt_of_src = (int*)take((size_t)max_voxels * 4);
  F.corr = (int*)take((size_t)max_voxels * 16);
  F.nc_cnt = (int*)take((size_t)max_voxels * 4);
  F.nc_fill = (int*)take((size_t)max_voxels * 4);
  F.nc_off = (int*)take((size_t)(max_voxels + 1) * 4);
  F.nc_list = (int*)take((size_t)max_voxels * 8);
  F.mcounts = (int*)take(16 * 4);
  F.nn_partial = take((((size_t)max_voxels + 511) / 512 * 512) * 32 * 16);
  F.recheck_rows = (int*)take((size_t)max_voxels * 4);
  F.recheck_thr = (float*)take((size_t)max_voxels * 4);
  F.recheck_span = (int2*)take((size_t)max_voxels * 8);
  F.hit_rows = (int*)take((size_t)max_voxels * 4);
  F.queryT_c = (float*)take(34 * (((size_t)max_voxels + 511) / 512 * 512) * 4);
  F.norms_c = (float*)take((((size_t)max_voxels + 511) / 512 * 512) * 4);
  F.queryH_c = (uint4*)take((((size_t)max_voxels + 511) / 512 * 512) * 224 + 2 * 7168);
  F.recheck_q = (int*)take((size_t)max_voxels * 4);
  {
    const char* e = QTR_ENGINE_ENV("QTR_NN_ENGINE");
    F.nn_engine = (e && strcmp(e, "exact") == 0) ? 0 : (e && strcmp(e, "mfma32") == 0) ? 1 : 2;
    int dev = 0, cus = 0;
    if (hipGetDevice(&dev) == hipSuccess &&
        hipDeviceGetAttribute(&cus, hipDeviceAttributeMultiprocessorCount, dev) == hipSuccess && cus > 0)
      F.n_cu = cus;
  }
}

hipError_t match_init_attributes();
hipError_t frontend_init_attributes() {
  hipError_t e;
  if ((e = hipFuncSetAttribute((const void*)k2_neighbors_big<false>, hipFuncAttributeMaxDynamicSharedMemorySize,
                               NBIG_LDS_KEYS * 8)) != hipSuccess)
    return e;
  if ((e = hipFuncSetAttribute((const void*)k2_neighbors_big<true>, hipFuncAttributeMaxDynamicSharedMemorySize,
                               NBIG_LDS_KEYS * 8)) != hipSuccess)
    return e;
  return match_init_attributes();
}
```

### quatro_amd/csrc/match.hip

```cpp
#include <vector>

#include "common.h"
#include "frontend.h"

#define NN_TILE 64
#define CROSS_LDS_BYTES (156 * 1024)
#define NN_STRIDE 36

#define LAUNCH_MV_K(kern, K, a, grid, block, lds, st, ...)                                                       \
  do {                                                                                                          \
    if ((a).ext)                                                                                                \
      hipLaunchKernelGGL((kern<true, K>), grid, block, lds, st, (ViewExt<MatchView>{(a).ext, {0, 0, 0}}), (a).one, ##__VA_ARGS__); \
    else                                                                                                        \
      hipLaunchKernelGGL((kern<false, K>), grid, block, lds, st, (ViewExt<MatchView>{nullptr, {0, 0, 0}}), (a).one, ##__VA_ARGS__); \
  } while (0)
#define LAUNCH_MV_EV(kern, a, grid, block, lds, st, e0, e1, ...)                                                 \
  do {                                                                                                          \
    if ((a).ext)                                                                                                \
      hipExtLaunchKernelGGL((kern<true>), grid, block, lds, st, e0, e1, 0, (ViewExt<MatchView>{(a).ext, {0, 0, 0}}), (a).one, ##__VA_ARGS__);  \
    else                                                                                                        \
      hipExtLaunchKernelGGL((kern<false>), grid, block, lds, st, e0, e1, 0, (ViewExt<MatchView>{nullptr, {0, 0, 0}}), (a).one, ##__VA_ARGS__); \
  } while (0)
#define LAUNCH_MV(kern, a, grid, block, lds, st, ...)                                       \
  do {                                                                                      \
// ... 1184 lines not shown
      const int ri = g * XR + r;
      const float val = (ri < nrows) ? A[(size_t)rows[ri] * 33 + k] : 0.f;
      s_a[r][k] = val;
      s_m2a[k][r] = -2.0f * val;
    }
    if (threadIdx.x < XR) {
      const int ri = g * XR + threadIdx.x;
      s_row[threadIdx.x] = (ri < nrows) ? rows[ri] : -1;
      s_thr[threadIdx.x] = (ri < nrows) ? thr[ri] : -INFINITY;
      s_best[threadIdx.x] = ~0ULL;
    }
    if (threadIdx.x == 64) {
      int lo = 0x7fffffff, hi = 0;
      for (int r = 0; r < XR; ++r) {
        const int ri = g * XR + r;
        if (ri < nrows) {
          const int2 sp = span[ri];
          lo = min(lo, sp.x);
          hi = max(hi, sp.y);
        }
      }
      s_span[0] = lo;
      s_span[1] = hi;
    }
    __syncthreads();
    const int per = (max(s_span[1] - s_span[0], 0) + gridDim.y - 1) / gridDim.y;
    const int b0 = s_span[0] + blockIdx.y * per, b1 = min(s_span[1], b0 + per);
    for (int b = b0 + wave * 64 + lane; b < b1; b += 256) {
      asm volatile("" ::: "memory");
      float v[34];
      const u32 bu = (u32)b;
#pragma unroll
      for (int k = 0; k < 34; ++k) v[k] = (BT + (size_t)k * nb_pad)[bu];
      float ap[XR];
#pragma unroll
      for (int r = 0; r < XR; ++r) ap[r] = v[33];
#pragma unroll
      for (int k = 0; k < 33; ++k) {
        if (k % 4 == 0) asm volatile("" ::: "memory");
        const float4 ma = *(const float4*)&s_m2a[k][0], mb = *(const float4*)&s_m2a[k][4];
        ap[0] = fmaf(ma.x, v[k], ap[0]);
        ap[1] = fmaf(ma.y, v[k], ap[1]);
        ap[2] = fmaf(ma.z, v[k], ap[2]);
        ap[3] = fmaf(ma.w, v[k], ap[3]);
        ap[4] = fmaf(mb.x, v[k], ap[4]);
        ap[5] = fmaf(mb.y, v[k], ap[5]);
        ap[6] = fmaf(mb.z, v[k], ap[6]);
        ap[7] = fmaf(mb.w, v[k], ap[7]);
      }
      u32 pass = 0;
#pragma unroll
      for (int r = 0; r < XR; ++r) pass |= (ap[r] <= s_thr[r]) ? (1u << r) : 0u;
      while (pass) {
        const int r = __ffs((int)pass) - 1;
        pass &= pass - 1;
        const float* av = s_a[r];
        float result = 0.f;
#pragma unroll
        for (int q4 = 0; q4 < 8; ++q4) {
          const float4 a4 = *(const float4*)(av + 4 * q4);
          const float d0 = a4.x - v[4 * q4], d1 = a4.y - v[4 * q4 + 1], d2 = a4.z - v[4 * q4 + 2],
                      d3 = a4.w - v[4 * q4 + 3];
          result += d0 * d0 + d1 * d1 + d2 * d2 + d3 * d3;
        }
        const float dt = av[32] - v[32];
        result += dt * dt;
        atomicMin(&s_best[r], ((u64)__float_as_uint(result) << 32) | (u32)brow[b]);
      }
    }
    __syncthreads();
    if (threadIdx.x < XR && s_row[threadIdx.x] >= 0 && s_best[threadIdx.x] != ~0ULL)
      atomicMin(&best[s_row[threadIdx.x]], s_best[threadIdx.x]);
  }
}

template <bool EXT>
__global__ __launch_bounds__(256) void k_match_init(ViewExt<MatchView> x, MatchView one, int clear_tables, int* zero_words,
                                                    int n_zero) {
  const MatchView& V = EXT ? x.ext[blockIdx.z] : one;
  const int gid = blockIdx.x * blockDim.x + threadIdx.x, gsz = gridDim.x * blockDim.x;
  if (zero_words && blockIdx.x == gridDim.x - 1 && blockIdx.z == 0)
    for (int i = threadIdx.x; i < n_zero; i += blockDim.x) zero_words[i] = 0;
  if (gid < 16) V.mcounts[gid] = (gid == MC_SWAPPED) ? V.swapped : (gid == MC_NQ0) ? V.n_small : 0;
  const int pv = V.tuple ? 0 : 1;
  const int np = V.crosscheck ? V.n_small : V.n_small + V.n_large;
  for (int i = gid; i < np; i += gsz) V.passed[i] = pv;
  if (!V.crosscheck)
    for (int i = gid; i < V.ns; i += gsz) V.nc_cnt[i] = V.nc_fill[i] = 0;
  for (int i = gid; i < V.ns; i += gsz) V.tgt_of_src[i] = -1;
  for (int i = gid; i < V.n_small; i += gsz) V.best_small[i] = ~0ULL;
  for (int i = gid; i < V.n_large; i += gsz) V.best_large[i] = ~0ULL;
  if (clear_tables)
    for (int i = gid; i <= V.dd_mask; i += gsz) {
      V.table_i[i] = ~0ULL;
      V.table_j[i] = ~0ULL;
    }
  for (int i = gid; i < 2 * TAIL_MAXWG; i += gsz) V.scan[i] = 0;
}

template <bool EXT>
__global__ __launch_bounds__(1024) void k_hit_compact(ViewExt<MatchView> x, MatchView one, int bin_order, int nn_X) {
  const MatchView& V = EXT ? x.ext[blockIdx.z] : one;
  extern __shared__ u32 hit_bits[];
  __shared__ int wsum[16];
  const int tid = threadIdx.x, lane = tid & 63, wave = tid >> 6;
  const int n = V.n_large, nw = (n + 31) / 32, ns = V.n_small;
  QTR_STAMP(STAMP_HIT_COMPACT, 0)
  for (int w = tid; w < nw; w += 1024) hit_bits[w] = 0u;
  __syncthreads();
  for (int j0 = tid; j0 < ns; j0 += 16 * 1024) {
    u64 b[16];
#pragma unroll
    for (int q = 0; q < 16; ++q) b[q] = (j0 + q * 1024 < ns) ? V.best_small[j0 + q * 1024] : 0ULL;
#pragma unroll
    for (int q = 0; q < 16; ++q)
      if (j0 + q * 1024 < ns) {
        const int i = (b[q] == ~0ULL) ? 0 : (int)(u32)b[q];
        atomicOr(&hit_bits[i >> 5], 1u << (i & 31));
      }
  }
  __syncthreads();
  QTR_STAMP(STAMP_HIT_COMPACT, 1)
  const int items = bin_order ? n : nw;
  const int per = (items + 1023) / 1024;
  const int p0 = min(items, tid * per), p1 = min(items, p0 + per);
  int cnt = 0;
  if (bin_order) {
    for (int p = p0; p < p1; ++p) {
      const int r = V.nb_row_i[p];
      cnt += (hit_bits[r >> 5] >> (r & 31)) & 1u;
    }
  } else {
    for (int w = p0; w < p1; ++w) cnt += __popc(hit_bits[w]);
  }
  int tot;
  const int ex = wave_excl_scan_i32(cnt, &tot);
  if (lane == 63) wsum[wave] = tot;
  __syncthreads();
  int run = ex, total = 0;
#pragma unroll
  for (int w = 0; w < 16; ++w) {
    run += (w < wave) ? wsum[w] : 0;
    total += wsum[w];
  }
  if (bin_order) {
    for (int p = p0; p < p1; ++p) {
      const int r = V.nb_row_i[p];
      if ((hit_bits[r >> 5] >> (r & 31)) & 1u) V.hit_rows[run++] = r;
    }
  } else {
    for (int w = p0; w < p1; ++w) {
      u32 bits = hit_bits[w];
      while (bits) {
        V.hit_rows[run++] = 32 * w + (__ffs((int)bits) - 1);
        bits &= bits - 1;
      }
    }
  }
  if (tid == 0) {
    V.mcounts[MC_NHIT] = total;
    if (nn_X > 0) V.mcounts[MC_NSPLIT1] = nn_plan_single((total + NN_QPB - 1) / NN_QPB, V.d[1].nb_pad / 32, nn_X);
  }
  QTR_STAMP(STAMP_HIT_COMPACT, 2)
}

template <bool EXT>
__global__ __launch_bounds__(256) void k_hit_gather(ViewExt<MatchView> x, MatchView one, int f32_tables) {
  const MatchView& V = EXT ? x.ext[blockIdx.z] : one;
  const int nhit = V.mcounts[MC_NHIT];
  const int padded = (nhit + NN_QPB - 1) / NN_QPB * NN_QPB;
  const int c = blockIdx.x * 256 + threadIdx.x;
  if (c >= padded) return;
  const int pad = V.pad_large;
  if (c < nhit) {
    const int r = V.hit_rows[c];
    V.norms_c[c] = V.norms_i[r];
    if (f32_tables) {
#pragma unroll
      for (int k = 0; k < 34; ++k) V.queryT_c[(size_t)k * pad + c] = V.queryT_i[(size_t)k * pad + r];
    } else {
#pragma unroll
      for (int ch = 0; ch < NNH_CHUNKS; ++ch)
        V.queryH_c[((size_t)(c >> 5) * NNH_CHUNKS + ch) * 32 + (c & 31)] = V.queryH_i[((size_t)(r >> 5) * NNH_CHUNKS + ch) * 32 + (r & 31)];
    }
  } else {
    V.norms_c[c] = 0.f;
    if (f32_tables) {
#pragma unroll
      for (int k = 0; k < 33; ++k) V.queryT_c[(size_t)k * pad + c] = 0.f;
      V.queryT_c[(size_t)33 * pad + c] = 1.0f;
    } else {
#pragma unroll
      for (int ch = 0; ch < NNH_CHUNKS; ++ch) V.queryH_c[((size_t)(c >> 5) * NNH_CHUNKS + ch) * 32 + (c & 31)] = make_uint4(0, 0, 0, 0);
    }
  }
}

template <bool EXT>
__global__ __launch_bounds__(256) void k_cross_flags2(ViewExt<MatchView> x, MatchView one) {
  const MatchView& V = EXT ? x.ext[blockIdx.z] : one;
  const int gid = blockIdx.x * blockDim.x + threadIdx.x, gsz = gridDim.x * blockDim.x;
  for (int j = gid; j < V.n_small; j += gsz) {
    const u64 b = V.best_small[j];
    V.nn_of_small[j] = (b == ~0ULL) ? 0 : (int)(u32)b;
  }
  for (int i = gid; i < V.n_large; i += gsz) {
    const u64 b = V.best_large[i];
    const int j = (b == ~0ULL) ? 0 : (int)(u32)b;
    V.nn_of_large[i] = (b == ~0ULL) ? -1 : j;
    const u64 bs = V.best_small[j];
    const int back = (bs == ~0ULL) ? 0 : (int)(u32)bs;
    V.flags[i] = V.crosscheck ? ((b != ~0ULL && back == i) ? 1 : 0) : ((b != ~0ULL) ? 1 : 0);
  }
}

template <bool EXT>
__global__ __launch_bounds__(1024) void k_scan_flags(ViewExt<MatchView> x, MatchView one) {
  const MatchView& V = EXT ? x.ext[blockIdx.z] : one;
  d_block_scan(V.flags, V.scan, V.n_large, [](int x) { return x; });
}
template <bool EXT>
__global__ __launch_bounds__(1024) void k_scan_nonneg(ViewExt<MatchView> x, MatchView one) {
  const MatchView& V = EXT ? x.ext[blockIdx.z] : one;
  d_block_scan(V.tgt_of_src, V.scan, V.ns, [](int x) { return x >= 0 ? 1 : 0; });
}

__device__ __forceinline__ void match_mail(const MatchView& V, int t, int total, int ntuple) {
  int* mail = V.mail;
  if (t < 16)
    mail_store_line(mail + MAIL_MATCH, t, (t == MC_NCORR) ? total : (t == MC_NTUPLE) ? ntuple : V.mcounts[t], V.seq);
  else if (t < 32)
    mail_store_line(mail + MAIL_CNT0, t - 16, V.counts0[t - 16], V.seq);
  else
    mail_store_line(mail + MAIL_CNT1, t - 32, V.counts1[t - 32], V.seq);
  __threadfence_system();
  if (t == 0) mail[MAIL_SEQ_MATCH] = V.seq;
}

template <bool EXT>
__global__ void k_corr_compact2(ViewExt<MatchView> x, MatchView one) {
  const MatchView& V = EXT ? x.ext[blockIdx.z] : one;
  const int ns = V.ns;
  for (int s = blockIdx.x * blockDim.x + threadIdx.x; s < ns; s += gridDim.x * blockDim.x) {
    const int t = V.tgt_of_src[s];
    if (t >= 0) {
      V.corr[2 * V.scan[s]] = s;
      V.corr[2 * V.scan[s] + 1] = t;
    }
  }
  if (blockIdx.x == 0 && threadIdx.x == 0) V.mcounts[MC_NCORR] = V.scan[ns];
  if (V.mail && blockIdx.x == 0 && threadIdx.x < 48) match_mail(V, threadIdx.x, V.scan[ns], V.mcounts[MC_NTUPLE]);
}

template <bool EXT>
__global__ void k_cross_compact(ViewExt<MatchView> x, MatchView one) {
  const MatchView& V = EXT ? x.ext[blockIdx.z] : one;
  for (int i = blockIdx.x * blockDim.x + threadIdx.x; i < V.n_large; i += gridDim.x * blockDim.x) {
    if (V.flags[i]) {
      V.cross_i[V.scan[i]] = i;
      V.cross_j[V.scan[i]] = V.nn_of_large[i];
    }
  }
  if (blockIdx.x == 0 && threadIdx.x == 0) V.mcounts[MC_NCROSS] = V.scan[V.n_large];
}

template <bool EXT>
__global__ __launch_bounds__(256) void k_tuple(ViewExt<MatchView> x, MatchView one) {
  const MatchView& V = EXT ? x.ext[blockIdx.z] : one;
  if (!V.tuple) return;
  const int ncorr = V.mcounts[MC_NCROSS];
  if (ncorr <= 0) return;
  const float4* __restrict__ pts_i = V.vox_i;
  const float4* __restrict__ pts_j = V.vox_j;
  const int* __restrict__ cross_i = V.cross_i;
  const int* __restrict__ cross_j = V.cross_j;
  const float scale = V.tuple_scale;
  const u64 seed = V.seed;
  const long long trials = (long long)ncorr * 100;
  const float mix = V.mean_i[0], miy = V.mean_i[1], miz = V.mean_i[2];
  const float mjx = V.mean_j[0], mjy = V.mean_j[1], mjz = V.mean_j[2];
  for (long long t = (long long)blockIdx.x * blockDim.x + threadIdx.x; t < trials;
       t += (long long)gridDim.x * blockDim.x) {
    const int r0 = (int)(qm_rand_u32(seed, 3ULL * (u64)t) % (u32)ncorr);
    const int r1 = (int)(qm_rand_u32(seed, 3ULL * (u64)t + 1ULL) % (u32)ncorr);
    const int r2 = (int)(qm_rand_u32(seed, 3ULL * (u64)t + 2ULL) % (u32)ncorr);
    float pi[3][3], pj[3][3];
    const int rr[3] = {r0, r1, r2};
#pragma unroll
    for (int k = 0; k < 3; ++k) {
      const float4 pa = pts_i[cross_i[rr[k]]], pb = pts_j[cross_j[rr[k]]];
      pi[k][0] = pa.x - mix;
      pi[k][1] = pa.y - miy;
      pi[k][2] = pa.z - miz;
      pj[k][0] = pb.x - mjx;
      pj[k][1] = pb.y - mjy;
      pj[k][2] = pb.z - mjz;
    }
    float li[3], lj[3];
#pragma unroll
    for (int k = 0; k < 3; ++k) {
      const int k2 = (k + 1) % 3;
      float dx = pi[k][0] - pi[k2][0], dy = pi[k][1] - pi[k2][1], dz = pi[k][2] - pi[k2][2];
      li[k] = sqrtf(dx * dx + (dy * dy + dz * dz));
      dx = pj[k][0] - pj[k2][0];
      dy = pj[k][1] - pj[k2][1];
      dz = pj[k][2] - pj[k2][2];
      lj[k] = sqrtf(dx * dx + (dy * dy + dz * dz));
    }
    if ((li[0] * scale < lj[0]) && (lj[0] < li[0] / scale) && (li[1] * scale < lj[1]) && (lj[1] < li[1] / scale) &&
        (li[2] * scale < lj[2]) && (lj[2] < li[2] / scale)) {
      V.passed[r0] = 1;
      V.passed[r1] = 1;
      V.passed[r2] = 1;
    }
  }
}

template <bool EXT>
__global__ void k_scatter_pairs(ViewExt<MatchView> x, MatchView one) {
// ... 247 lines not shown
    total += wsum[w];
  }
#pragma unroll
  for (int k = 0; k < KMAX; ++k)
    if ((keep >> k) & 1u) {
      V.cross_i[run] = base + k;
      V.cross_j[run] = jj[k];
      ++run;
    }
  if (tid == 0) V.mcounts[MC_NCROSS] = total;
  QTR_STAMP(STAMP_CROSS, 2)
}

template <bool EXT, int KMAX>
__global__ __launch_bounds__(1024) void k_pairs_fused(ViewExt<MatchView> x, MatchView one) {
  const MatchView& V = EXT ? x.ext[blockIdx.z] : one;
  __shared__ int wsum[16];
  __shared__ int s_ntuple;
  extern __shared__ int tg_s[];
  const int tid = threadIdx.x, lane = tid & 63, wave = tid >> 6;
  const int swapped = V.swapped, ns = V.ns;
  if (tid == 0) s_ntuple = 0;
  for (int i = tid; i < ns; i += 1024) tg_s[i] = -1;
  __syncthreads();
  const int nc = V.mcounts[MC_NCROSS];
  int local = 0;
  for (int c0 = tid; c0 < nc; c0 += 8 * 1024) {
    int pf[8], ci[8], cj[8];
#pragma unroll
    for (int q = 0; q < 8; ++q) {
      const int c = min(c0 + q * 1024, nc - 1);
      pf[q] = (c0 + q * 1024 < nc) ? (int)V.passed[c] : 0;
      ci[q] = V.cross_i[c];
      cj[q] = V.cross_j[c];
    }
#pragma unroll
    for (int q = 0; q < 8; ++q)
      if (pf[q]) {
        tg_s[swapped ? cj[q] : ci[q]] = swapped ? ci[q] : cj[q];
        ++local;
      }
  }
  local = wave_sum_i32(local);
  if (lane == 0 && local) atomicAdd(&s_ntuple, local);
  __syncthreads();
  const int K = (ns + 1023) >> 10, base = tid * K;
  int tt[KMAX];
  int cnt = 0;
#pragma unroll
  for (int k = 0; k < KMAX; ++k) {
    const int sidx = base + k;
    tt[k] = (k < K && sidx < ns) ? tg_s[sidx] : -1;
    cnt += tt[k] >= 0 ? 1 : 0;
  }
  int tot;
  const int ex = wave_excl_scan_i32(cnt, &tot);
  if (lane == 63) wsum[wave] = tot;
  __syncthreads();
  int run = ex, total = 0;
#pragma unroll
  for (int w = 0; w < 16; ++w) {
    run += (w < wave) ? wsum[w] : 0;
    total += wsum[w];
  }
  if (V.mail && tid < 48) match_mail(V, tid, total, s_ntuple);
#pragma unroll
  for (int k = 0; k < KMAX; ++k)
    if (tt[k] >= 0) {
      V.corr[2 * run] = base + k;
      V.corr[2 * run + 1] = tt[k];
      if (V.m_src && run < V.m_cap) {
        float4 pa = V.vox_s[base + k], pb = V.vox_t[tt[k]];
        pa.w = 0.f;
        pb.w = 0.f;
        V.m_src[run] = pa;
        V.m_tgt[run] = pb;
      }
      ++run;
    }
  if (tid == 0) {
    V.mcounts[MC_NCORR] = total;
    V.mcounts[MC_NTUPLE] = s_ntuple;
  }
}

#define CM_ROWS 512
template <bool EXT>
__global__ __launch_bounds__(256) void k_cross_multi(ViewExt<MatchView> x, MatchView one) {
  const MatchView& V = EXT ? x.ext[blockIdx.z] : one;
  const int n_large = V.n_large, n_small = V.n_small;
  const int nwg = (n_large + CM_ROWS - 1) / CM_ROWS, w = blockIdx.x;
  if (w >= nwg) return;
  __shared__ int s_w[4], s_red[5];
  const int tid = threadIdx.x, lane = tid & 63, wave = tid >> 6;
  {
    const int per = (n_small + nwg - 1) / nwg, j0 = w * per, j1 = min(n_small, j0 + per);
    for (int j = j0 + tid; j < j1; j += 256) {
      const u64 bsm = V.best_small[j];
      V.nn_of_small[j] = (bsm == ~0ULL) ? 0 : (int)(u32)bsm;
    }
  }
  const int base = w * CM_ROWS + 2 * tid;
  u64 b[2], bs[2];
  int jj[2];
#pragma unroll
  for (int k = 0; k < 2; ++k) b[k] = (base + k < n_large) ? V.best_large[base + k] : ~0ULL;
#pragma unroll
  for (int k = 0; k < 2; ++k) {
    jj[k] = (b[k] == ~0ULL) ? 0 : (int)(u32)b[k];
    bs[k] = V.best_small[jj[k]];
  }
  bool keep[2];
  int cnt = 0;
#pragma unroll
  for (int k = 0; k < 2; ++k) {
    const int i = base + k;
    const int back = (bs[k] == ~0ULL) ? 0 : (int)(u32)bs[k];
    keep[k] = i < n_large && b[k] != ~0ULL && back == i;
    if (i < n_large) V.nn_of_large[i] = (b[k] == ~0ULL) ? -1 : jj[k];
    cnt += keep[k] ? 1 : 0;
  }
  int tot;
  const int ex = wave_excl_scan_i32(cnt, &tot);
  if (lane == 0) s_w[wave] = tot;
  __syncthreads();
  int run = ex, total = 0;
#pragma unroll
  for (int q = 0; q < 4; ++q) {
    run += (q < wave) ? s_w[q] : 0;
    total += s_w[q];
  }
  const int before = tail_lookback(V.scan, w, total, s_red);
  if (before < 0) {
    if (tid == 0) {
      V.mcounts[MC_TAILERR] = 1;
      if (w == nwg - 1) V.mcounts[MC_NCROSS] = 0;
    }
    return;
  }
  run += before;
#pragma unroll
  for (int k = 0; k < 2; ++k)
    if (keep[k]) {
      V.cross_i[run] = base + k;
      V.cross_j[run] = jj[k];
      ++run;
    }
  if (w == nwg - 1 && tid == 0) V.mcounts[MC_NCROSS] = before + total;
}

#define PM_SRC 512
template <bool EXT>
__global__ __launch_bounds__(256) void k_pairs_multi(ViewExt<MatchView> x, MatchView one) {
  const MatchView& V = EXT ? x.ext[blockIdx.z] : one;
  const int ns = V.ns, swapped = V.swapped;
  const int nwg = max(1, (ns + PM_SRC - 1) / PM_SRC), w = blockIdx.x;
  if (w >= nwg) return;
  __shared__ int s_tg[PM_SRC];
  __shared__ int s_w[4], s_red[5], s_ntuple;
  const int tid = threadIdx.x, lane = tid & 63, wave = tid >> 6;
  const int s0 = w * PM_SRC;
  s_tg[2 * tid] = -1;
  s_tg[2 * tid + 1] = -1;
  if (tid == 0) s_ntuple = 0;
  __syncthreads();
  const int nc = V.mcounts[MC_NCROSS];
  int local = 0;
  for (int c0 = tid; c0 < nc; c0 += 8 * 256) {
    int pf[8], ci[8], cj[8];
#pragma unroll
    for (int q = 0; q < 8; ++q) {
      const int c = min(c0 + q * 256, nc - 1);
      pf[q] = (c0 + q * 256 < nc) ? (int)V.passed[c] : 0;
      ci[q] = V.cross_i[c];
      cj[q] = V.cross_j[c];
    }
#pragma unroll
    for (int q = 0; q < 8; ++q)
      if (pf[q]) {
        const int src = (swapped ? cj[q] : ci[q]) - s0;
        if (src >= 0 && src < PM_SRC) s_tg[src] = swapped ? ci[q] : cj[q];
        ++local;
      }
  }
  local = wave_sum_i32(local);
  if (lane == 0 && local) atomicAdd(&s_ntuple, local);
  __syncthreads();
  int tt[2], cnt = 0;
#pragma unroll
  for (int k = 0; k < 2; ++k) {
    tt[k] = (s0 + 2 * tid + k < ns) ? s_tg[2 * tid + k] : -1;
    cnt += tt[k] >= 0 ? 1 : 0;
  }
  int tot;
  const int ex = wave_excl_scan_i32(cnt, &tot);
  if (lane == 0) s_w[wave] = tot;
  __syncthreads();
  int run = ex, total = 0;
#pragma unroll
  for (int q = 0; q < 4; ++q) {
    run += (q < wave) ? s_w[q] : 0;
    total += s_w[q];
  }
  const int before = tail_lookback(V.scan + TAIL_MAXWG, w, total, s_red);
  const bool tail_err = before < 0 || V.mcounts[MC_TAILERR] != 0;
  run += before;
  if (w == nwg - 1) {
    if (V.mail && tid < 48) match_mail(V, tid, tail_err ? -1 : before + total, s_ntuple);
    if (tid == 0) {
      V.mcounts[MC_NCORR] = tail_err ? -1 : before + total;
      V.mcounts[MC_NTUPLE] = s_ntuple;
    }
  }
  if (tail_err) return;
#pragma unroll
  for (int k = 0; k < 2; ++k)
    if (tt[k] >= 0) {
      const int src = s0 + 2 * tid + k;
      V.corr[2 * run] = src;
      V.corr[2 * run + 1] = tt[k];
      if (V.m_src && run < V.m_cap) {
        float4 pa = V.vox_s[src], pb = V.vox_t[tt[k]];
        pa.w = 0.f;
        pb.w = 0.f;
        V.m_src[run] = pa;
        V.m_tgt[run] = pb;
      }
      ++run;
    }
}

__global__ void k_gather_matched(const float4* __restrict__ vs, const float4* __restrict__ vt,
                                 const int* __restrict__ corr, int L, float4* __restrict__ ms, float4* __restrict__ mt) {
  for (int c = blockIdx.x * blockDim.x + threadIdx.x; c < L; c += gridDim.x * blockDim.x) {
    float4 a = vs[corr[2 * c]], b = vt[corr[2 * c + 1]];
    a.w = 0.f;
    b.w = 0.f;
    ms[c] = a;
    mt[c] = b;
  }
}

static_assert(CM_ROWS == 512 && PM_SRC == 512, "TAIL_MAXWG look-back words cover TAIL_MAXWG * 512 rows");
static bool tail_is_fused(bool crosscheck, int max_large, int max_ns) {
  static const bool tail_single = [] {
    const char* e = QTR_ENGINE_ENV("QTR_MATCH_TAIL");
    return e && strcmp(e, "single") == 0;
  }();
  const int lim = tail_single ? 32768 : TAIL_MAXWG * 512;
  return crosscheck && max_large <= lim && max_ns <= lim;
}
static inline int grid_for(int n) {
  int g = (n + 255) / 256;
  return g < 1 ? 1 : (g > 2048 ? 2048 : g);
}

static MatchView make_match_view(FrontBufs& F, int ns, int nt, const qtr_frontend_params& fp, unsigned long long seed) {
  MatchView V;
  memset(&V, 0, sizeof(V));
  const int swapped = nt > ns ? 1 : 0;
  CloudBufs& Ci = F.cloud[swapped ? 1 : 0];
  CloudBufs& Cj = F.cloud[swapped ? 0 : 1];
  V.swapped = swapped;
  V.ns = ns;
  V.nt = nt;
  V.n_large = swapped ? nt : ns;
  V.n_small = swapped ? ns : nt;
  V.pad_large = (V.n_large + NN_QPB - 1) / NN_QPB * NN_QPB;
  V.pad_small = (V.n_small + NN_QPB - 1) / NN_QPB * NN_QPB;
  V.vox_i = Ci.vox;
  V.vox_j = Cj.vox;
  V.mean_i = Ci.mean;
  V.mean_j = Cj.mean;
  V.fpfh_i = Ci.fpfh;
  V.fpfh_j = Cj.fpfh;
  V.baseT_i = Ci.baseT;
  V.queryT_i = Ci.queryT;
  V.norms_i = Ci.norms;
  V.baseT_j = Cj.baseT;
  V.queryT_j = Cj.queryT;
  V.norms_j = Cj.norms;
  V.baseTb_i = Ci.baseTb;
  V.baseTb_j = Cj.baseTb;
  V.baseH_i = Ci.baseH;
  V.baseH_j = Cj.baseH;
  V.queryH_i = Ci.queryH;
  V.queryH_j = Cj.queryH;
  V.queryH_c = F.queryH_c;
  V.nb_row_i = Ci.nb_row;
  V.nb_row_j = Cj.nb_row;
  V.nb_start_i = Ci.nb_start;
  V.nb_start_j = Cj.nb_start;
  V.hash_i = Ci.dd_hash;
  V.hash_j = Cj.dd_hash;
  V.table_i = Ci.dd_table;
  V.table_j = Cj.dd_table;
  V.dd_mask = F.dd_slots - 1;
  V.best_small = F.best_small;
  V.best_large = F.best_large;
  V.nn_of_small = F.nn_of_small;
  V.nn_of_large = F.nn_of_large;
  V.cross_i = F.cross_i;
  V.cross_j = F.cross_j;
  V.flags = F.flags;
  V.scan = F.scan;
  V.passed = F.passed;
  V.tgt_of_src = F.tgt_of_src;
  V.corr = F.corr;
  V.mcounts = F.mcounts;
  V.partial = (NnPartial*)F.nn_partial;
  V.recheck_rows = F.recheck_rows;
  V.recheck_thr = F.recheck_thr;
  V.recheck_span = F.recheck_span;
  V.recheck_q = F.recheck_q;
  V.hit_rows = F.hit_rows;
  V.queryT_c = F.queryT_c;
  V.norms_c = F.norms_c;
  V.vox_s = F.cloud[0].vox;
  V.vox_t = F.cloud[1].vox;
  V.m_src = F.m_src;
  V.m_tgt = F.m_tgt;
  V.m_cap = F.m_cap;
  V.mail = F.mail;
  V.counts0 = F.cloud[0].counts;
  V.counts1 = F.cloud[1].counts;
  V.seq = F.mail_seq;
  V.nc_cnt = F.nc_cnt;
  V.nc_fill = F.nc_fill;
  V.nc_off = F.nc_off;
  V.nc_list = F.nc_list;
  V.crosscheck = fp.use_crosscheck ? 1 : 0;
  V.tuple = (fp.use_tuple_test && fp.tuple_scale != 0) ? 1 : 0;
  V.tuple_scale = fp.tuple_scale;
  V.seed = seed;
// ... 144 lines not shown
      if (G > 1) ex = max(8, 384 / G);
#ifdef QTR_TEST_ENGINES
      if (!f16) LAUNCH_MV(k_nn_exact_rows, a, dim3(ex, ey, G), B256, 0, st, dir);
#else
      (void)ex;
      (void)ey;
#endif
    };
    run_dir(0, max_small, max_large, ev ? ev[0] : nullptr, ev ? ev[1] : nullptr);
    LAUNCH_MV(k_hit_compact, a, dim3(1, 1, G), dim3(1024), (size_t)((max_large + 31) / 32) * 4, st, f16 ? 0 : 1,
              (f16 && G == 1) ? X : 0);
#ifdef QTR_TEST_ENGINES
    if (!f16) LAUNCH_MV(k_hit_gather, a, dim3(max_pad / 256, 1, G), B256, 0, st, 1);
#endif
    run_dir(1, max_large, max_small, ev ? ev[2] : nullptr, ev ? ev[3] : nullptr);
  }
  const bool crosscheck = views[0].crosscheck != 0;
  const bool fused_tail = tail_is_fused(crosscheck, max_large, max_ns);
  const bool fused16 = max_large <= 16384 && max_ns <= 16384;
  static const bool tail_single = [] {
    const char* e = QTR_ENGINE_ENV("QTR_MATCH_TAIL");
    return e && strcmp(e, "single") == 0;
  }();
  const bool tail_multi = fused_tail && !tail_single;
  if (!crosscheck) {
    LAUNCH_MV(k_cross_flags2, a, dim3(grid_for(max_large), 1, G), B256, 0, st);
    LAUNCH_MV(k_scan_flags, a, dim3(1, 1, G), dim3(1024), 0, st);
    LAUNCH_MV(k_nc_list, a, dim3(grid_for(max_large + max_small), 1, G), B256, 0, st);
  } else if (fused_tail) {
    const int lds_gather = ((size_t)max_large + (size_t)max_small) * 4 <= (size_t)CROSS_LDS_BYTES ? 1 : 0;
    const size_t cross_lds = (size_t)max_large * 4 + (lds_gather ? (size_t)max_small * 4 : 0);
    if (tail_multi) LAUNCH_MV(k_cross_multi, a, dim3((max_large + CM_ROWS - 1) / CM_ROWS, 1, G), B256, 0, st);
#ifdef QTR_TEST_ENGINES
    else if (fused16) LAUNCH_MV_K(k_cross_fused, 16, a, dim3(1, 1, G), dim3(1024), cross_lds, st, lds_gather);
    else LAUNCH_MV_K(k_cross_fused, 32, a, dim3(1, 1, G), dim3(1024), cross_lds, st, lds_gather);
#else
    (void)cross_lds;
    (void)fused16;
#endif
  } else {
    LAUNCH_MV(k_cross_flags2, a, dim3(grid_for(max_large), 1, G), B256, 0, st);
    LAUNCH_MV(k_scan_flags, a, dim3(1, 1, G), dim3(1024), 0, st);
    LAUNCH_MV(k_cross_compact, a, dim3(grid_for(max_large), 1, G), B256, 0, st);
  }
  if (any_tuple) LAUNCH_MV(k_tuple, a, dim3(G > 1 ? 256 : 2048, 1, G), B256, 0, st);
  if (!crosscheck) {
    const int gl = grid_for(max_large + max_small), gs = grid_for(max_ns);
    LAUNCH_MV(k_nc_scatter, a, dim3(gl, 1, G), B256, 0, st, 0);
    LAUNCH_MV(k_nc_scan, a, dim3(1, 1, G), dim3(1024), 0, st, 0);
    LAUNCH_MV(k_nc_scatter, a, dim3(gl, 1, G), B256, 0, st, 1);
    LAUNCH_MV(k_nc_unique, a, dim3(gs, 1, G), B256, 0, st);
    LAUNCH_MV(k_nc_scan, a, dim3(1, 1, G), dim3(1024), 0, st, 1);
    LAUNCH_MV(k_nc_emit, a, dim3(gs, 1, G), B256, 0, st);
  } else if (fused_tail) {
    if (tail_multi) LAUNCH_MV(k_pairs_multi, a, dim3(max(1, (max_ns + PM_SRC - 1) / PM_SRC), 1, G), B256, 0, st);
#ifdef QTR_TEST_ENGINES
    else if (fused16) LAUNCH_MV_K(k_pairs_fused, 16, a, dim3(1, 1, G), dim3(1024), (size_t)max_ns * 4, st);
    else LAUNCH_MV_K(k_pairs_fused, 32, a, dim3(1, 1, G), dim3(1024), (size_t)max_ns * 4, st);
#endif
  } else {
    LAUNCH_MV(k_scatter_pairs, a, dim3(grid_for(max_small), 1, G), B256, 0, st);
    LAUNCH_MV(k_scan_nonneg, a, dim3(1, 1, G), dim3(1024), 0, st);
    LAUNCH_MV(k_corr_compact2, a, dim3(grid_for(max_ns), 1, G), B256, 0, st);
  }
  return hipGetLastError();
}

hipError_t match_init_enqueue(FrontBufs& F, int ns, int nt, const qtr_frontend_params& fp, hipStream_t st, bool clear_tables,
                              int* zero_words, int n_zero) {
  (void)hipGetLastError();
  MatchArgs a;
  a.one = make_match_view(F, ns, nt, fp, (unsigned long long)fp.seed);
  a.ext = nullptr;
  LAUNCH_MV(k_match_init, a, dim3(grid_for(max(a.one.n_large, a.one.dd_mask + 1)), 1, 1), dim3(256), 0, st, clear_tables ? 1 : 0, zero_words, n_zero);
  return hipGetLastError();
}
hipError_t match_enqueue(FrontBufs& F, int ns, int nt, const qtr_frontend_params& fp, hipStream_t st, bool init_done,
                         bool prep_done, bool gather) {
  (void)hipGetLastError();
  MatchView V = make_match_view(F, ns, nt, fp, (unsigned long long)fp.seed);
  if (!gather) V.m_src = V.m_tgt = nullptr;
  const bool fused_tail = tail_is_fused(V.crosscheck != 0, V.n_large, ns);
  F.gathered = fused_tail && V.m_src != nullptr;
  const bool evs = F.nn_events != 0;
  return match_launch(&V, 1, F.nn_engine, F.n_cu, nullptr, st, evs ? F.ev_nn : nullptr, init_done, prep_done);
}

hipError_t match_enqueue_group(FrontBufs* const* F, int G, const int* n, const qtr_frontend_params* fp,
                               const unsigned long long* seeds, ViewStage* stage, hipStream_t st, bool prep_done) {
  (void)hipGetLastError();
  std::vector<MatchView> v((size_t)G);
  int max_large = 1, max_ns = 1;
  for (int g = 0; g < G; ++g) {
    v[g] = make_match_view(*F[g], n[2 * g], n[2 * g + 1], *fp, seeds[g]);
    max_large = max(max_large, v[g].n_large);
    max_ns = max(max_ns, v[g].ns);
  }
  const bool fused_tail = tail_is_fused(fp->use_crosscheck != 0, max_large, max_ns);
  for (int g = 0; g < G; ++g) F[g]->gathered = fused_tail && F[g]->m_src != nullptr;
  return match_launch(v.data(), G, F[0]->nn_engine, F[0]->n_cu, stage, st, nullptr, false, prep_done);
}

hipError_t gather_matched_enqueue(FrontBufs& F, int L, float4* m_src, float4* m_tgt, hipStream_t st) {
  if (L <= 0 || (F.gathered && m_src == F.m_src && m_tgt == F.m_tgt)) return hipSuccess;
  hipLaunchKernelGGL(k_gather_matched, dim3(grid_for(L)), dim3(256), 0, st, F.cloud[0].vox, F.cloud[1].vox, F.corr, L,
                     m_src, m_tgt);
  return hipGetLastError();
}

hipError_t match_init_attributes() {
  hipError_t e;
  (void)e;
#ifdef QTR_TEST_ENGINES
  if ((e = hipFuncSetAttribute((const void*)k_cross_fused<false, 16>, hipFuncAttributeMaxDynamicSharedMemorySize, CROSS_LDS_BYTES)) != hipSuccess) return e;
  if ((e = hipFuncSetAttribute((const void*)k_cross_fused<true, 16>, hipFuncAttributeMaxDynamicSharedMemorySize, CROSS_LDS_BYTES)) != hipSuccess) return e;
  if ((e = hipFuncSetAttribute((const void*)k_cross_fused<false, 32>, hipFuncAttributeMaxDynamicSharedMemorySize, CROSS_LDS_BYTES)) != hipSuccess) return e;
  if ((e = hipFuncSetAttribute((const void*)k_cross_fused<true, 32>, hipFuncAttributeMaxDynamicSharedMemorySize, CROSS_LDS_BYTES)) != hipSuccess) return e;
#define SET_LDS2(kern)                                                                                                   \
  if ((e = hipFuncSetAttribute((const void*)kern<false, 32>, hipFuncAttributeMaxDynamicSharedMemorySize, 132 * 1024)) != hipSuccess) \
    return e;                                                                                                            \
  if ((e = hipFuncSetAttribute((const void*)kern<true, 32>, hipFuncAttributeMaxDynamicSharedMemorySize, 132 * 1024)) != hipSuccess)  \
    return e;
  SET_LDS2(k_pairs_fused)
#undef SET_LDS2
#endif
  return hipSuccess;
}
```

### quatro_amd/lib.py

```python
from __future__ import annotations

import ctypes as C
import os

import numpy as np

_HERE = os.path.dirname(os.path.abspath(__file__))
LIB_PATH = os.environ.get("QTR_LIB") or os.path.join(_HERE, "libquatro_hip.so")

QTR_OK, QTR_ERR_BAD_ARG, QTR_ERR_CLIQUE_TOO_SMALL, QTR_ERR_CAPACITY, QTR_ERR_HIP, QTR_ERR_UNSUPPORTED = range(6)
MEM_HOST, MEM_DEVICE = 0, 1
INLIER_PMC_EXACT, INLIER_PMC_HEU, INLIER_KCORE_HEU, INLIER_NONE = range(4)
REG_QUATRO, REG_TEASER = 0, 1

DBG_GRAPH_BITMAP, DBG_CORE, DBG_PERM, DBG_NBR_OFFSETS, DBG_NBR_INDEX, DBG_NBR_DIST2, DBG_SPFH = 1, 2, 3, 4, 5, 6, 7
DBG_NN_LARGE_OF_SMALL, DBG_NN_SMALL_OF_LARGE, DBG_VOX_SRC, DBG_VOX_TGT, DBG_CORR, DBG_MATCH_STATS = 8, 9, 10, 11, 12, 13
DBG_SOLVER_STATE = 14
DBG_ICP_CORR, DBG_ICP_TRACE, DBG_ICP_TIMES = 15, 16, 17
ICP_POINT_TO_PLANE, ICP_POINT_TO_POINT, ICP_PLANE_TO_PLANE, ICP_VOXEL_PLANE_TO_PLANE = 0, 1, 2, 3
ICP_STOP_NONE, ICP_STOP_MAX_ITERATIONS, ICP_STOP_TRANSFORMATION, ICP_STOP_FITNESS, ICP_STOP_TOO_FEW, ICP_STOP_DEGENERATE = range(6)


class Limits(C.Structure):
    _fields_ = [("max_points", C.c_int), ("max_voxels", C.c_int), ("max_corr", C.c_int), ("n_slots", C.c_int),
# ... 56 lines not shown
class IcpParams(C.Structure):
    _fields_ = [("max_correspondence_distance", C.c_double), ("transformation_epsilon", C.c_double),
                ("euclidean_fitness_epsilon", C.c_double), ("max_iterations", C.c_int), ("method", C.c_int),
                ("min_correspondences", C.c_int), ("normal_radius", C.c_float)]


class IcpResult(C.Structure):
    _fields_ = [("status", C.c_int), ("valid", C.c_int), ("converged", C.c_int), ("stop_reason", C.c_int),
                ("iterations", C.c_int), ("n_corr", C.c_int), ("T", C.c_double * 16), ("fitness", C.c_double),
                ("rmse", C.c_double)]


class EvalParams(C.Structure):
    _fields_ = [("max_correspondence_distance", C.c_double), ("reserved", C.c_int * 2)]


class EvalResult(C.Structure):
    _fields_ = [("status", C.c_int), ("valid", C.c_int), ("n_source", C.c_int), ("n_corr", C.c_int), ("n_plane", C.c_int),
                ("reserved", C.c_int), ("T", C.c_double * 16), ("overlap", C.c_double), ("sum_d2", C.c_double),
                ("inlier_rmse", C.c_double), ("plane_rmse", C.c_double), ("information", C.c_double * 36),
                ("hessian_plane", C.c_double * 36)]


class EvalKfPair(C.Structure):
    _fields_ = [("source", C.c_void_p), ("target", C.c_void_p), ("T", C.c_double * 16)]


class PgoParams(C.Structure):
    _fields_ = [("max_iterations", C.c_int), ("pcg_max_iterations", C.c_int), ("rel_tol", C.c_double),
                ("step_tol", C.c_double), ("tau", C.c_double), ("pcg_tol", C.c_double),
                ("line_process_weight", C.c_double), ("edge_prune_threshold", C.c_double), ("reserved", C.c_int * 8)]


class PgoResult(C.Structure):
    _fields_ = [("status", C.c_int), ("valid", C.c_int), ("iterations", C.c_int), ("accepted", C.c_int),
                ("pcg_iterations_total", C.c_int), ("stop_reason", C.c_int), ("n_pruned", C.c_int), ("reserved", C.c_int),
                ("objective_initial", C.c_double), ("objective_final", C.c_double), ("lambda_final", C.c_double)]


class KeyframeInfo(C.Structure):
    _fields_ = [("n_points", C.c_int), ("n_voxels", C.c_int), ("voxel_size", C.c_float), ("normal_radius", C.c_float),
                ("fpfh_radius", C.c_float), ("passed_through", C.c_int), ("device_bytes", C.c_ulonglong)]


class KfPairDesc(C.Structure):
    _fields_ = [("src", C.c_void_p), ("tgt", C.c_void_p), ("seed", C.c_ulonglong), ("clique", C.c_void_p),
                ("final_inliers", C.c_void_p), ("cap", C.c_int)]


class PlaceParams(C.Structure):
    _fields_ = [("num_rings", C.c_int), ("num_sectors", C.c_int), ("max_range", C.c_float), ("height_offset", C.c_float)]


class PlaceMatch(C.Structure):
    _fields_ = [("id", C.c_int), ("shift", C.c_int), ("distance", C.c_float), ("yaw", C.c_float)]


class PlaceIndexInfo(C.Structure):
    _fields_ = [("params", PlaceParams), ("size", C.c_int), ("capacity", C.c_int), ("device_bytes", C.c_ulonglong)]


class VoxelMapParams(C.Structure):
    _fields_ = [("voxel_size", C.c_double), ("capacity", C.c_int), ("reserved", C.c_int * 5)]


class VoxelMapInfo(C.Structure):
    _fields_ = [("voxel_size", C.c_double), ("capacity", C.c_int), ("n_voxels", C.c_int), ("n_inserts", C.c_int),
                ("n_members", C.c_longlong)]


class VoxelMapInsertInfo(C.Structure):
    _fields_ = [("n_points", C.c_int), ("n_members", C.c_int), ("n_new_voxels", C.c_int), ("n_touched_voxels", C.c_int)]


KF_VOX, KF_NORMALS, KF_FPFH, KF_MEAN = 1, 2, 3, 4
VMAP_COORDS, VMAP_COUNT, VMAP_SUMS, VMAP_RECORDS, VMAP_CLOUD = 1, 2, 3, 4, 5
VMAP_MAX_CAPACITY = 1 << 24
PLACE_DESC, PLACE_COLNORM2 = 1, 2
PLACE_MAX_K = 64
SUBMAP_MAX_KEYFRAMES = 64
EVAL_MAX_PAIRS = 64
DBG_EVAL_CORR = 18
DBG_PGO_TRACE = 19
PGO_MAX_NODES, PGO_MAX_EDGES, PGO_MAX_ITERATIONS, PGO_TRACE = 65536, 1 << 20, 65536, 8
PGO_STOP_MAX_ITERATIONS, PGO_STOP_RELATIVE, PGO_STOP_STEP, PGO_STOP_LAMBDA, PGO_STOP_NOTHING = 1, 2, 3, 4, 5

EXPORTS = [
    "qtr_create", "qtr_destroy", "qtr_last_error", "qtr_default_limits", "qtr_default_params", "qtr_demo_params",
    "qtr_default_frontend_params", "qtr_num_slots", "qtr_slot_stream", "qtr_voxelize", "qtr_fpfh", "qtr_match",
    "qtr_solve", "qtr_max_clique", "qtr_compute_tims", "qtr_scale_mask", "qtr_gnc_rotation2d",
    "qtr_cote_estimate", "qtr_cote_estimate_ranges", "qtr_ip_default_params", "qtr_segment_cloud", "qtr_pw_default_params", "qtr_patchwork", "qtr_gnc_rotation3d", "qtr_exact_stats", "qtr_read_kitti_bin", "qtr_write_pcd_xyz", "qtr_read_pcd_xyz", "qtr_register_pair", "qtr_register_pair_corr", "qtr_feature_pair", "qtr_get_stage_times", "qtr_get_nn_dir_times", "qtr_set_stage_events", "qtr_set_nn_event_stride", "qtr_get_nn_totals", "qtr_debug_fetch", "qtr_debug_math", "qtr_submit_batch", "qtr_wait", "qtr_set_batch_preprocess", "qtr_comm_unique_id", "qtr_comm_init", "qtr_gather_results", "qtr_gather_results_v", "qtr_comm_destroy",
    "qtr_default_icp_params", "qtr_icp", "qtr_refine_pair", "qtr_submit_batch_refine", "qtr_gicp",
    "qtr_keyframe_create", "qtr_keyframe_get_info", "qtr_keyframe_fetch", "qtr_keyframe_destroy", "qtr_register_keyframes",
    "qtr_submit_batch_keyframes", "qtr_keyframe_merge",
    "qtr_default_place_params", "qtr_place_index_create", "qtr_place_index_destroy", "qtr_place_index_get_info",
    "qtr_place_describe", "qtr_place_index_add", "qtr_place_index_add_desc", "qtr_place_index_fetch", "qtr_place_query",
    "qtr_place_query_desc",
    "qtr_default_eval_params", "qtr_evaluate", "qtr_evaluate_pair", "qtr_evaluate_keyframes",
    "qtr_evaluate_keyframes_batch",
    "qtr_default_pgo_params", "qtr_pgo_optimize",
]
VOXELMAP_EXPORTS = [
    "qtr_default_voxel_map_params", "qtr_voxel_map_create", "qtr_voxel_map_destroy", "qtr_voxel_map_clear",
    "qtr_voxel_map_get_info", "qtr_voxel_map_insert", "qtr_voxel_map_insert_keyframe", "qtr_voxel_map_register",
    "qtr_voxel_map_register_keyframe", "qtr_voxel_map_fetch",
]

_lib = None


QTR_ERR_IO = 6
QTR_ERR_NOT_RUN = 7


def read_kitti_bin(path: str, max_points: int = 250000) -> np.ndarray:
    out = np.zeros((max(max_points, 1), 4), dtype=np.float32)
    n = C.c_int()
    rc = load().qtr_read_kitti_bin(os.fsencode(path), out.ctypes.data, max_points, C.byref(n))
    if rc != QTR_OK:
        raise OSError(f"error: failed to load {path}")
    return out[:n.value].copy()


def write_pcd_xyz(path: str, xyz, binary: bool = False) -> None:
    a = np.asarray(xyz, dtype=np.float32).reshape(-1, np.asarray(xyz).shape[-1] if np.asarray(xyz).ndim == 2 else 3)
    if a.shape[1] == 3:
        a = np.concatenate([a, np.zeros((a.shape[0], 1), dtype=np.float32)], axis=1)
    a = _f4(a[:, :4])
    rc = load().qtr_write_pcd_xyz(os.fsencode(path), a.ctypes.data, a.shape[0], 1 if binary else 0)
    if rc != QTR_OK:
        raise OSError(f"failed to write {path}")


def read_pcd_xyz(path: str) -> np.ndarray:
    n = C.c_int()
    rc = load().qtr_read_pcd_xyz(os.fsencode(path), None, 0, C.byref(n))
    if rc not in (QTR_OK, QTR_ERR_CAPACITY):
        raise OSError(f"failed to read {path}")
    out = np.zeros((max(n.value, 1), 4), dtype=np.float32)
    rc = load().qtr_read_pcd_xyz(os.fsencode(path), out.ctypes.data, n.value, C.byref(n))
    if rc != QTR_OK:
        raise OSError(f"failed to read {path}")
    return out[:n.value].copy()


def pw_params() -> PwParams:
    p = PwParams()
    load().qtr_pw_default_params(C.byref(p))
    return p


def ip_params(lidar: str = "Velodyne-64-HDE", neighbor_mode: str = "4CrossNeighbor", num_min_pts: int = 30) -> IpParams:
    p = IpParams()
    rc = load().qtr_ip_default_params(lidar.encode(), neighbor_mode.encode(), C.byref(p))
    if rc != QTR_OK:
        raise ValueError("[ImageProjection]:Check your paramter. Lidar Type / neighbor selection mode is wrong!")
    p.num_min_pts = num_min_pts
    return p


class QuatroHipError(RuntimeError):
    def __init__(self, code: int, msg: str):
        super().__init__(f"libquatro_hip status {code}: {msg}")
        self.code = code


# ... 1127 lines not shown
```

Measured before the change: 3004 registrations/s.

## Handle solver follow-up during matcher wait and end call on mailbox done flag

The corr-overlap path now does its solver follow-up and stream join while the host is still waiting for the matcher, if the solver mail has already arrived. The final stream synchronize at the end of the call is replaced by a spin on a new mailbox word. The last matcher tail workgroup writes that word once all workgroups finish, using an atomic counter. This is meant to cut host-side latency and synchronize overhead per registration, at the cost of more mailbox protocol complexity and reliance on the done word covering all outstanding work. Host timestamps and a profiling script are added as test-build diagnostics.

```diff
diff --git a/include/quatro_hip.h b/include/quatro_hip.h
--- a/include/quatro_hip.h
+++ b/include/quatro_hip.h
@@ -392,6 +392,8 @@
 #define QTR_DBG_ICP_TIMES 17
 #define QTR_DBG_EVAL_CORR 18
 #define QTR_DBG_PGO_TRACE 19
+#define QTR_DBG_HOST_STAMPS 20
+#define QTR_DBG_STREAMS_IDLE 21
 QTR_API long long qtr_debug_fetch(qtr_handle* h, int slot, int what, void* dst, size_t bytes);
 
 QTR_API int qtr_debug_math(qtr_handle* h, int fn, const float* a, const float* b, float* out, int n);
diff --git a/profiles/end_wait_host.py b/profiles/end_wait_host.py
--- /dev/null
+++ b/profiles/end_wait_host.py
@@ -0,0 +1,98 @@
+from __future__ import annotations
+
+import argparse
+import os
+import sys
+import time
+
+import numpy as np
+
+ROOT = os.path.dirname(os.path.dirname(os.path.abspath(__file__)))
+if ROOT not in sys.path:
+    sys.path.insert(0, ROOT)
+
+NAMES = ("entry", "first launch issued", "voxel mail seen", "matcher enqueued", "matcher mail seen",
+         "solver mail handled", "join issued", "end-of-call wait returned")
+
+
+def main() -> None:
+    ap = argparse.ArgumentParser()
+    ap.add_argument("--lib", default=None, help="the test build (default: quatro_amd/libquatro_hip_testengines.so)")
+    ap.add_argument("--steps", type=int, default=400)
+    ap.add_argument("--warmup", type=int, default=20)
+    ap.add_argument("--label", default="")
+    ap.add_argument("--out", default=None)
+    args = ap.parse_args()
+
+    import torch
+    from quatro_amd import build as qbuild
+    from quatro_amd import lib as ql
+    from quatro_amd import synth
+
+    torch.cuda.set_device(0)
+    dev = torch.device("cuda", 0)
+    LC = 5000
+    ql.LIB_PATH = os.path.abspath(args.lib or qbuild.TEST_LIB)
+    h = ql.Handle(0, max_points=131072, max_voxels=32768, max_corr=8192, lib_path=ql.LIB_PATH)
+    prm = ql.demo_params()
+    res = ql.Result()
+    pool = []
+    for pid in range(4):
+        s, t, _ = synth.kitti64_pair_16k(pid)
+        cs, ct, _, _ = synth.correspondences(LC, 0.05, seed=pid, noise=0.1)
+        ten = [torch.from_numpy(a).to(dev) for a in (s, t, cs, ct)]
+        pool.append((ten, ql.default_frontend_params(seed=pid)))
+    torch.cuda.synchronize()
+
+    def step(p):
+        (s, t, cs, ct), fp = p
+        rc = h.register_pair_corr_dev(s.data_ptr(), int(s.shape[0]), t.data_ptr(), int(t.shape[0]), fp, cs.data_ptr(),
+                                      ct.data_ptr(), LC, prm, res)
+        if rc not in (ql.QTR_OK, ql.QTR_ERR_CLIQUE_TOO_SMALL):
+            raise ql.QuatroHipError(rc, h.last_error())
+
+    t_settle = time.perf_counter() + 0.25
+    k = 0
+    while time.perf_counter() < t_settle:
+        step(pool[k % 4])
+        k += 1
+    for w in range(args.warmup):
+        step(pool[w % 4])
+    torch.cuda.synchronize()
+    h.set_stage_events(False)
+    h.set_nn_event_stride(5)
+    stamps = np.zeros((args.steps, 8))
+    back = np.zeros(args.steps)
+    t0 = time.perf_counter()
+    for i in range(args.steps):
+        a = time.perf_counter()
+        step(pool[i % 4])
+        back[i] = time.perf_counter() - a
+        stamps[i] = h.debug_fetch(ql.DBG_HOST_STAMPS, np.float64)
+    torch.cuda.synchronize()
+    wall = time.perf_counter() - t0
+    d = np.diff(stamps, axis=1)
+    lines = [f"host timeline of the headline step{(' -- ' + args.label) if args.label else ''}",
+             f"{args.steps} steps after {args.warmup} warm-up steps, test build, microseconds (median | 10th .. 90th percentile)",
+             f"loop: {1e3 * wall / args.steps:.4f} ms per step including the stamp read-back; the call itself: median "
+             f"{1e6 * np.median(back):.1f} us", ""]
+    for j in range(7):
+        q = np.percentile(d[:, j], (50, 10, 90))
+        lines.append(f"  {NAMES[j]:>26} -> {NAMES[j + 1]:<26} {q[0]:8.2f} | {q[1]:8.2f} .. {q[2]:8.2f}")
+    post = stamps[:, 7] - stamps[:, 4]
+    q = np.percentile(post, (50, 10, 90))
+    lines.append("")
+    lines.append(f"  matcher mail seen -> return (post-mail host work + join + end-of-call wait): {q[0]:.2f} | {q[1]:.2f} .. {q[2]:.2f}")
+    q = np.percentile(stamps[:, 7] - stamps[:, 0], (50, 10, 90))
+    lines.append(f"  entry -> return: {q[0]:.2f} | {q[1]:.2f} .. {q[2]:.2f}")
+    text = "\n".join(lines) + "\n"
+    print(text, end="")
+    if args.out:
+        os.makedirs(os.path.dirname(os.path.abspath(args.out)), exist_ok=True)
+        with open(args.out, "w") as f:
+            f.write(text)
+    h.close()
+
+
+if __name__ == "__main__":
+    main()
diff --git a/quatro_amd/csrc/capi.hip b/quatro_amd/csrc/capi.hip
--- a/quatro_amd/csrc/capi.hip
+++ b/quatro_amd/csrc/capi.hip
@@ -2,6 +2,7 @@
 
 #include <algorithm>
 #include <atomic>
+#include <chrono>
 #include <memory>
 #include <mutex>
 #include <new>
@@ -15,6 +16,14 @@
 struct RcclIdByValue {
   char internal[QTR_COMM_ID_BYTES];
 };
+
+enum { HS_ENTRY = 0, HS_FIRST_LAUNCH, HS_VOX_MAIL, HS_MATCH_ENQ, HS_MATCH_MAIL, HS_SOLVE_MAIL, HS_JOIN, HS_DRAIN, HS_N };
+#ifdef QTR_TEST_ENGINES
+#define QTR_HSTAMP(s, k)                                                                                                \
+  ((s).hstamp[k] = std::chrono::duration<double, std::micro>(std::chrono::steady_clock::now().time_since_epoch()).count())
+#else
+#define QTR_HSTAMP(s, k) ((void)0)
+#endif
 
 struct Slot {
   hipStream_t stream = nullptr;
@@ -45,6 +54,7 @@
   void* pw_arena = nullptr;
   int* mail = nullptr;
   int seq = 0;
+  int match_seq = 0;
   unsigned long long exact_nodes = 0;
   int exact_aborted = 0;
   int times_pending = 0;
@@ -69,6 +79,10 @@
   PlaceScratch place;
   KfGatherMember* merge_pin = nullptr;
   KfGatherMember* merge_dev = nullptr;
+#ifdef QTR_TEST_ENGINES
+  double hstamp[HS_N] = {};
+#endif
+  int streams_idle[3] = {};
 };
 
 enum LanePhase { LANE_IDLE = 0, LANE_VOXELS, LANE_MATCH, LANE_SOLVE, LANE_REFINE_BOXES, LANE_REFINE_ITER };
@@ -610,6 +624,7 @@
     case MAIL_SEQ_VOX0: return line_ok(MAIL_VOX0);
     case MAIL_SEQ_VOX1: return line_ok(MAIL_VOX1);
     case MAIL_SEQ_MATCH: return line_ok(MAIL_MATCH) && line_ok(MAIL_CNT0) && line_ok(MAIL_CNT1);
+    case MAIL_SEQ_MATCH_DONE: return line_ok(MAIL_MATCH_DONE);
     case MAIL_SEQ_SOLVE: return solver_ok();
     case MAIL_SEQ_ICP_BOX: return line_ok(MAIL_ICP_BOX);
     case MAIL_SEQ_ICP: return line_ok(MAIL_ICP) && line_ok(MAIL_ICP + 16) && line_ok(MAIL_ICP + 32);
@@ -928,13 +943,14 @@
   return wait_mail(h, s, MAIL_SEQ_SOLVE, s.seq);
 }
 
-static void result_from_mail(const Slot& s, qtr_result* res) {
+static void result_from_record(const void* rec, qtr_result* res) {
   const int keep_ns = res->n_src, keep_nt = res->n_tgt, keep_nc = res->n_corr;
-  memcpy(res, s.mail + MAIL_SOLVER, sizeof(qtr_result));
+  memcpy(res, rec, sizeof(qtr_result));
   res->n_src = keep_ns;
   res->n_tgt = keep_nt;
   res->n_corr = keep_nc;
 }
+static void result_from_mail(const Slot& s, qtr_result* res) { result_from_record(s.mail + MAIL_SOLVER, res); }
 
 static int corr_stage(qtr_handle* h, Slot& s, const float* src4, const float* tgt4, int n, int mem, hipStream_t st,
                       const float4** cs, const float4** ct) {
@@ -984,6 +1000,18 @@
   return QTR_OK;
 }
 
+static int finish_call(qtr_handle* h, Slot& s, const qtr_result* res, int* clique, int* rot_inliers, int* final_inliers,
+                       int cap, int mem, bool host_inputs, int match_done_seq) {
+  if (!h->spin_wait || host_inputs || clique || rot_inliers || final_inliers)
+    return copy_out_lists(h, s, res, clique, rot_inliers, final_inliers, cap, mem);
+  if (!match_done_seq) return QTR_OK;
+  if (!s.fb.tail_done_word) {
+    QTR_HIP_TRY(h, hipStreamSynchronize(s.stream));
+    return QTR_OK;
+  }
+  return wait_mail(h, s, MAIL_SEQ_MATCH_DONE, match_done_seq);
+}
+
 int qtr_solve(qtr_handle* h, int slot, const float* src4, const float* tgt4, int L, const qtr_params* prm,
               qtr_result* res, int* clique, int* rot_inliers, int* final_inliers, int cap, int mem) {
   Slot* sp = get_slot(h, slot);
@@ -1007,7 +1035,7 @@
   rc = solve_device(h, s, d_src, d_tgt, L, prm, res);
   if (rc != QTR_OK && rc != QTR_ERR_CLIQUE_TOO_SMALL) return rc;
   s.times_pending = ev_on ? 1 : 4;
-  const int rc2 = copy_out_lists(h, s, res, clique, rot_inliers, final_inliers, cap, mem);
+  const int rc2 = finish_call(h, s, res, clique, rot_inliers, final_inliers, cap, mem, mem == QTR_MEM_HOST, 0);
   if (rc2 != QTR_OK) return res->status = rc2;
   return rc;
 }
@@ -1592,16 +1620,23 @@
   return QTR_OK;
 }
 
+struct CorrEarly;
+static void corr_paperwork(qtr_handle* h, Slot& s, CorrEarly& ce, bool at_the_end);
+
 static int match_device(qtr_handle* h, Slot& s, int ns, int nt, const qtr_frontend_params* fp, int* L_out,
-                        bool init_done = false, bool prep_done = false, bool tolerate_tail = false, bool gather = true) {
+                        bool init_done = false, bool prep_done = false, bool tolerate_tail = false, bool gather = true,
+                        CorrEarly* early = nullptr) {
   flush_nn_totals(s);
   const int stride = h->nn_event_stride;
   s.fb.nn_events = (stride > 0 && (s.n_matches++ % stride) == 0) ? 1 : 0;
   s.nn_timed_last = (s.fb.nn_events && s.fb.nn_engine != 0) ? 1 : 0;
   s.nn_pending = s.nn_timed_last;
-  s.fb.mail_seq = ++s.seq;
+  const int match_seq = s.match_seq = s.fb.mail_seq = ++s.seq;
   QTR_HIP_TRY(h, match_enqueue(s.fb, ns, nt, *fp, s.stream, init_done, prep_done, gather));
-  QTR_TRY(wait_mail(h, s, MAIL_SEQ_MATCH, s.seq));
+  QTR_HSTAMP(s, HS_MATCH_ENQ);
+  if (early) corr_paperwork(h, s, *early, false);
+  QTR_TRY(wait_mail(h, s, MAIL_SEQ_MATCH, match_seq));
+  QTR_HSTAMP(s, HS_MATCH_MAIL);
   *L_out = s.mail[MAIL_MATCH + MC_NCORR];
   if (*L_out < 0) {
     if (tolerate_tail) return QTR_OK;
@@ -1677,6 +1712,9 @@
   int seq = 0;
   const float4 *cs = nullptr, *ct = nullptr;
   std::unique_ptr<InFlight> in_flight;
+  bool handled = false;
+  int paper_rc = QTR_OK;
+  qtr_result rec;
 };
 static int corr_early_enqueue(qtr_handle* h, Slot& s, CorrEarly& ce) {
   ce.enqueued = true;
@@ -1694,6 +1732,31 @@
   return QTR_OK;
 }
 
+struct StreamSwap {
+  Slot& s;
+  hipStream_t keep;
+  StreamSwap(Slot& s_, hipStream_t st) : s(s_), keep(s_.stream) { s.stream = st; }
+  ~StreamSwap() { s.stream = keep; }
+};
+
+static void corr_paperwork(qtr_handle* h, Slot& s, CorrEarly& ce, bool at_the_end) {
+  if (ce.handled || !ce.enqueued) return;
+  if (!at_the_end && (!h->spin_wait || !mail_ready(s, MAIL_SEQ_SOLVE, ce.seq))) return;
+  ce.handled = true;
+  ce.paper_rc = [&]() -> int {
+    StreamSwap on_stream3(s, s.stream3);
+    QTR_TRY(wait_mail(h, s, MAIL_SEQ_SOLVE, ce.seq));
+    QTR_TRY(solve_followup(h, s, ce.cs, ce.ct, ce.n, ce.prm, s.stream3, h->stage_events != 0));
+    ce.in_flight.reset();
+    memcpy(&ce.rec, s.mail + MAIL_SOLVER, sizeof(qtr_result));
+    QTR_HSTAMP(s, HS_SOLVE_MAIL);
+    QTR_HIP_TRY(h, hipEventRecord(s.ev_join, s.stream3));
+    QTR_HIP_TRY(h, hipStreamWaitEvent(on_stream3.keep, s.ev_join, 0));
+    QTR_HSTAMP(s, HS_JOIN);
+    return QTR_OK;
+  }();
+}
+
 static int front_device(qtr_handle* h, Slot& s, const float* src_raw4, int Ps, const float* tgt_raw4, int Pt,
                         const qtr_frontend_params* fp, int mem, bool for_solver, int* ns_out, int* nt_out, int* L_out,
                         bool corr_given = false, CorrEarly* early = nullptr) {
@@ -1725,6 +1788,7 @@
   if (h->stage_events) QTR_HIP_TRY(h, hipEventRecord(s.ev[0], s.stream));
   auto fail_drained = [&](int code) {
     (void)hipStreamSynchronize(s.stream);
+    (void)hipStreamSynchronize(s.stream2);
     return code;
   };
   {
@@ -1734,6 +1798,7 @@
       const int launched = s.fb.vox_passes;
       const int vox_seq = s.fb.mail_seq = ++s.seq;
       QTR_HIP_TRY(h, voxelize_enqueue(s.fb, 2, raws, Ps2, fp->voxel_size, s.stream, launched, fp->fpfh_radius * 1.001f));
+      if (attempt == 0) QTR_HSTAMP(s, HS_FIRST_LAUNCH);
       QTR_HIP_TRY(h, hipEventRecord(s.ev_vox, s.stream));
       {
         const int on_device[2] = {-1, -1};
@@ -1743,6 +1808,7 @@
       if (early && !early->enqueued) QTR_TRY(corr_early_enqueue(h, s, *early));
       if ((rc = wait_mail(h, s, MAIL_SEQ_VOX0, vox_seq)) != QTR_OK || (rc = wait_mail(h, s, MAIL_SEQ_VOX1, vox_seq)) != QTR_OK)
         return fail_drained(rc);
+      QTR_HSTAMP(s, HS_VOX_MAIL);
       const int bits = std::max(s.mail[MAIL_VOX0 + CNT_SORT_BITS], s.mail[MAIL_VOX1 + CNT_SORT_BITS]);
       if (!vox_passes_next(s.fb.vox_passes, s.fb.vox_fewer, bits, launched, attempt)) break;
     }
@@ -1788,7 +1854,7 @@
   }
   if (h->stage_events) QTR_HIP_TRY(h, hipEventRecord(s.ev[6], s.stream));
   int L = 0;
-  rc = match_device(h, s, ns, nt, fp, &L, true, true, corr_given, early == nullptr);
+  rc = match_device(h, s, ns, nt, fp, &L, true, true, corr_given, early == nullptr, early);
   if (rc != QTR_OK) return rc;
   switch (lists_verdict(s.mail + MAIL_CNT0, s.mail + MAIL_CNT1, h->long_lists)) {
     case LISTS_TILE_ERROR:
@@ -1828,6 +1894,7 @@
                               const float* corr_tgt, int n_corr, int* n_matched = nullptr) {
   const bool given = n_corr >= 0;
   int L = 0;
+  QTR_HSTAMP(s, HS_ENTRY);
   if (given && h->corr_overlap) {
     CorrEarly ce;
     ce.src = corr_src;
@@ -1846,29 +1913,21 @@
         if (armed) (void)hipStreamSynchronize(st);
       }
     } drain{s.stream3};
-    struct StreamSwap {
-      Slot& s;
-      hipStream_t keep;
-      StreamSwap(Slot& s_, hipStream_t st) : s(s_), keep(s_.stream) { s.stream = st; }
-      ~StreamSwap() { s.stream = keep; }
-    };
     if (rc == QTR_OK) {
-      StreamSwap on_stream3(s, s.stream3);
-      rc = wait_mail(h, s, MAIL_SEQ_SOLVE, ce.seq);
-      if (rc == QTR_OK) rc = solve_followup(h, s, ce.cs, ce.ct, n_corr, prm, s.stream3, h->stage_events != 0);
+      corr_paperwork(h, s, ce, true);
+      rc = ce.paper_rc;
     }
     if (rc != QTR_OK) {
       return res->status = rc;
     }
-    ce.in_flight.reset();
-    result_from_mail(s, res);
+    result_from_record(&ce.rec, res);
     rc = res->status;
-    QTR_HIP_TRY(h, hipEventRecord(s.ev_join, s.stream3));
-    QTR_HIP_TRY(h, hipStreamWaitEvent(s.stream, s.ev_join, 0));
     if (h->stage_events) QTR_HIP_TRY(h, hipEventRecord(s.ev_end, s.stream));
     if (rc != QTR_OK && rc != QTR_ERR_CLIQUE_TOO_SMALL) return rc;
     s.times_pending = h->stage_events ? 6 : 4;
-    const int rc2 = copy_out_lists(h, s, res, clique, nullptr, final_inliers, cap, mem_out);
+    const int rc2 = finish_call(h, s, res, clique, nullptr, final_inliers, cap, mem_out,
+                                mem_in == QTR_MEM_HOST || mem_out == QTR_MEM_HOST, s.match_seq);
+    QTR_HSTAMP(s, HS_DRAIN);
     if (rc2 != QTR_OK) return res->status = rc2;
     drain.armed = false;
     return rc;
@@ -1880,9 +1939,13 @@
   const float4 *cs = s.m_src, *ct = s.m_tgt;
   if (given) QTR_TRY(corr_stage(h, s, corr_src, corr_tgt, n_corr, mem_out, s.stream, &cs, &ct));
   rc = solve_device(h, s, cs, ct, res->n_corr, prm, res, true);
+  QTR_HSTAMP(s, HS_SOLVE_MAIL);
+  QTR_HSTAMP(s, HS_JOIN);
   if (rc != QTR_OK && rc != QTR_ERR_CLIQUE_TOO_SMALL) return rc;
   s.times_pending = h->stage_events ? 2 : 4;
-  const int rc2 = copy_out_lists(h, s, res, clique, nullptr, final_inliers, cap, mem_out);
+  const int rc2 = finish_call(h, s, res, clique, nullptr, final_inliers, cap, mem_out,
+                              mem_in == QTR_MEM_HOST || (given && mem_out == QTR_MEM_HOST), 0);
+  QTR_HSTAMP(s, HS_DRAIN);
   if (rc2 != QTR_OK) return res->status = rc2;
   return rc;
 }
@@ -2489,7 +2552,7 @@
   rc = solve_device(h, s, s.m_src, s.m_tgt, L, prm, res, true);
   if (rc != QTR_OK && rc != QTR_ERR_CLIQUE_TOO_SMALL) return rc;
   s.times_pending = h->stage_events ? 5 : 4;
-  const int rc2 = copy_out_lists(h, s, res, clique, nullptr, final_inliers, cap, QTR_MEM_HOST);
+  const int rc2 = finish_call(h, s, res, clique, nullptr, final_inliers, cap, QTR_MEM_HOST, false, 0);
   if (rc2 != QTR_OK) return res->status = rc2;
   mark_registration(s, rc, res);
   return rc;
@@ -3959,10 +4022,26 @@
     case QTR_DBG_ICP_TIMES: src = s.icp_ms; have = sizeof(s.icp_ms); break;
     case QTR_DBG_EVAL_CORR: src = s.eval.last_corr; have = s.eval.last_corr ? (size_t)s.eval.last_ns * 4 : 0; break;
     case QTR_DBG_PGO_TRACE: src = s.pgo.last_trace; have = s.pgo.last_trace ? (size_t)s.pgo.last_rows * QTR_PGO_TRACE * 8 : 0; break;
+#ifdef QTR_TEST_ENGINES
+    case QTR_DBG_HOST_STAMPS: src = s.hstamp; have = sizeof(s.hstamp); break;
+#endif
+    case QTR_DBG_STREAMS_IDLE: {
+      const hipStream_t st[3] = {s.stream, s.stream2, s.stream3};
+      for (int k = 0; k < 3; ++k) {
+        const hipError_t q = st[k] ? hipStreamQuery(st[k]) : hipErrorInvalidHandle;
+        s.streams_idle[k] = !st[k] ? -1 : q == hipSuccess ? 1 : q == hipErrorNotReady ? 0 : -2;
+      }
+      (void)hipGetLastError();
+      src = s.streams_idle;
+      have = sizeof(s.streams_idle);
+      break;
+    }
     default: return -1;
   }
   const size_t n = have < bytes ? have : bytes;
-  if (dst && n > 0) {
+  if (dst && n > 0 && (what == QTR_DBG_HOST_STAMPS || what == QTR_DBG_STREAMS_IDLE)) {
+    memcpy(dst, src, n);
+  } else if (dst && n > 0) {
     if (hipStreamSynchronize(s.stream) != hipSuccess) return -1;
     if (what == QTR_DBG_GRAPH_BITMAP && s.last_Wb > W) {
       const size_t rows = n / ((size_t)W * 8);
diff --git a/quatro_amd/csrc/frontend.h b/quatro_amd/csrc/frontend.h
--- a/quatro_amd/csrc/frontend.h
+++ b/quatro_amd/csrc/frontend.h
@@ -12,10 +12,13 @@
 enum { MC_NCORR = 0, MC_HIDDEN_I = 1, MC_HIDDEN_J = 2, MC_NCROSS = 3, MC_NTUPLE = 4, MC_SWAPPED = 5, MC_NQ0 = 6, MC_NHIT = 7,
        MC_RECHECK0 = 8, MC_RECHECK1 = 9, MC_NSPLIT0 = 10, MC_NSPLIT1 = 11 ,
        MC_UNSAFE = 12,
-       MC_TAILERR = 13  };
+       MC_TAILERR = 13 ,
+       MC_DONE = 16 ,
+       MC_WORDS = 32 };
 
 enum { MAIL_VOX0 = 0, MAIL_VOX1 = 16, MAIL_MATCH = 32, MAIL_CNT0 = 48, MAIL_CNT1 = 64, MAIL_SEQ_VOX0 = 96, MAIL_SEQ_VOX1 = 97,
-       MAIL_SEQ_MATCH = 98, MAIL_SEQ_SOLVE = 99, MAIL_SEQ_ICP_BOX = 100, MAIL_SEQ_ICP = 101, MAIL_SOLVER = 128,
+       MAIL_SEQ_MATCH = 98, MAIL_SEQ_SOLVE = 99, MAIL_SEQ_ICP_BOX = 100, MAIL_SEQ_ICP = 101, MAIL_SEQ_MATCH_DONE = 102,
+       MAIL_MATCH_DONE = 112, MAIL_SOLVER = 128,
        MAIL_ICP_BOX = 256, MAIL_ICP = 272, MAIL_INTS = 512 };
 
 struct CloudBufs {
@@ -196,6 +199,7 @@
   int vox_passes = 4;
   int vox_fewer = 0;
   bool gathered = false;
+  bool tail_done_word = false;
   int mail_seq = 0;
   int nn_engine = 2;
   int n_cu = 256;
diff --git a/quatro_amd/csrc/frontend.hip b/quatro_amd/csrc/frontend.hip
--- a/quatro_amd/csrc/frontend.hip
+++ b/quatro_amd/csrc/frontend.hip
@@ -1814,7 +1814,7 @@
   F.nc_fill = (int*)take((size_t)max_voxels * 4);
   F.nc_off = (int*)take((size_t)(max_voxels + 1) * 4);
   F.nc_list = (int*)take((size_t)max_voxels * 8);
-  F.mcounts = (int*)take(16 * 4);
+  F.mcounts = (int*)take(MC_WORDS * 4);
   F.nn_partial = take((((size_t)max_voxels + 511) / 512 * 512) * 32 * 16);
   F.recheck_rows = (int*)take((size_t)max_voxels * 4);
   F.recheck_thr = (float*)take((size_t)max_voxels * 4);
diff --git a/quatro_amd/csrc/match.hip b/quatro_amd/csrc/match.hip
--- a/quatro_amd/csrc/match.hip
+++ b/quatro_amd/csrc/match.hip
@@ -1290,6 +1290,7 @@
   if (zero_words && blockIdx.x == gridDim.x - 1 && blockIdx.z == 0)
     for (int i = threadIdx.x; i < n_zero; i += blockDim.x) zero_words[i] = 0;
   if (gid < 16) V.mcounts[gid] = (gid == MC_SWAPPED) ? V.swapped : (gid == MC_NQ0) ? V.n_small : 0;
+  if (gid == MC_DONE) V.mcounts[MC_DONE] = 0;
   const int pv = V.tuple ? 0 : 1;
   const int np = V.crosscheck ? V.n_small : V.n_small + V.n_large;
   for (int i = gid; i < np; i += gsz) V.passed[i] = pv;
@@ -1443,6 +1444,21 @@
     mail_store_line(mail + MAIL_CNT1, t - 32, V.counts1[t - 32], V.seq);
   __threadfence_system();
   if (t == 0) mail[MAIL_SEQ_MATCH] = V.seq;
+}
+
+__device__ __forceinline__ void match_done(const MatchView& V, int nwg) {
+  if (!V.mail) return;
+  __shared__ int s_last;
+  __threadfence();
+  __syncthreads();
+  if (threadIdx.x == 0)
+    s_last = __hip_atomic_fetch_add(V.mcounts + MC_DONE, 1, __ATOMIC_ACQ_REL, __HIP_MEMORY_SCOPE_AGENT) == nwg - 1 ? 1 : 0;
+  __syncthreads();
+  if (s_last && threadIdx.x < 16) {
+    mail_store_line(V.mail + MAIL_MATCH_DONE, threadIdx.x, threadIdx.x == 0 ? nwg : 0, V.seq);
+    __threadfence_system();
+    if (threadIdx.x == 0) V.mail[MAIL_SEQ_MATCH_DONE] = V.seq;
+  }
 }
 
 template <bool EXT>
@@ -1856,6 +1872,7 @@
     V.mcounts[MC_NCORR] = total;
     V.mcounts[MC_NTUPLE] = s_ntuple;
   }
+  match_done(V, 1);
 }
 
 #define CM_ROWS 512
@@ -1986,10 +2003,9 @@
       V.mcounts[MC_NTUPLE] = s_ntuple;
     }
   }
-  if (tail_err) return;
 #pragma unroll
   for (int k = 0; k < 2; ++k)
-    if (tt[k] >= 0) {
+    if (!tail_err && tt[k] >= 0) {
       const int src = s0 + 2 * tid + k;
       V.corr[2 * run] = src;
       V.corr[2 * run + 1] = tt[k];
@@ -2002,6 +2018,7 @@
       }
       ++run;
     }
+  match_done(V, nwg);
 }
 
 __global__ void k_gather_matched(const float4* __restrict__ vs, const float4* __restrict__ vt,
@@ -2024,6 +2041,7 @@
   const int lim = tail_single ? 32768 : TAIL_MAXWG * 512;
   return crosscheck && max_large <= lim && max_ns <= lim;
 }
+static bool tail_publishes_done(bool crosscheck, int max_large, int max_ns) { return tail_is_fused(crosscheck, max_large, max_ns); }
 static inline int grid_for(int n) {
   int g = (n + 255) / 256;
   return g < 1 ? 1 : (g > 2048 ? 2048 : g);
@@ -2334,6 +2352,7 @@
   if (!gather) V.m_src = V.m_tgt = nullptr;
   const bool fused_tail = tail_is_fused(V.crosscheck != 0, V.n_large, ns);
   F.gathered = fused_tail && V.m_src != nullptr;
+  F.tail_done_word = F.mail != nullptr && tail_publishes_done(V.crosscheck != 0, V.n_large, ns);
   const bool evs = F.nn_events != 0;
   return match_launch(&V, 1, F.nn_engine, F.n_cu, nullptr, st, evs ? F.ev_nn : nullptr, init_done, prep_done);
 }
diff --git a/quatro_amd/lib.py b/quatro_amd/lib.py
--- a/quatro_amd/lib.py
+++ b/quatro_amd/lib.py
@@ -162,6 +162,8 @@
 EVAL_MAX_PAIRS = 64
 DBG_EVAL_CORR = 18
 DBG_PGO_TRACE = 19
+DBG_HOST_STAMPS = 20
+DBG_STREAMS_IDLE = 21
 PGO_MAX_NODES, PGO_MAX_EDGES, PGO_MAX_ITERATIONS, PGO_TRACE = 65536, 1 << 20, 65536, 8
 PGO_STOP_MAX_ITERATIONS, PGO_STOP_RELATIVE, PGO_STOP_STEP, PGO_STOP_LAMBDA, PGO_STOP_NOTHING = 1, 2, 3, 4, 5
 
```

New measurement: 3053 registrations/s, median of 6. About the same (+1.6%).
